# JokerJohn/DCReg

Hardware: AMD Instinct MI355X
Metric: ICP iterations/sec (higher is better)
Workload: dtype f64

## Files before the change

dcreg_amd/api.py:

```python
import ctypes as C
import math
import os

import numpy as np

_HERE = os.path.dirname(os.path.abspath(__file__))
LIB_PATH = os.environ.get("DCREG_LIB") or os.path.join(_HERE, "lib", "libdcreg_hip.so")

DETECTION = {"NONE_DETE": 0, "SCHUR_CONDITION_NUMBER": 1, "FULL_EVD_MIN_EIGENVALUE": 2,
             "EVD_SUB_CONDITION": 3, "FULL_SVD_CONDITION": 4}
HANDLING = {"NONE_HAND": 0, "STANDARD_REGULARIZATION": 1, "ADAPTIVE_REGULARIZATION": 2,
            "PRECONDITIONED_CG": 3, "SOLUTION_REMAPPING": 4, "TRUNCATED_SVD": 5}
METHODS = {
    "ME-SR": ("FULL_EVD_MIN_EIGENVALUE", "SOLUTION_REMAPPING"),
    "ME-TSVD": ("FULL_EVD_MIN_EIGENVALUE", "TRUNCATED_SVD"),
    "ME-TReg": ("FULL_EVD_MIN_EIGENVALUE", "STANDARD_REGULARIZATION"),
    "FCN-SR": ("FULL_SVD_CONDITION", "SOLUTION_REMAPPING"),
    "Ours": ("SCHUR_CONDITION_NUMBER", "PRECONDITIONED_CG"),
    "NONE": ("NONE_DETE", "NONE_HAND"),
}

OK, E_INVALID, E_NOMEM, E_DEVICE, E_STATE = 0, -1, -2, -3, -4
ROBUST = {"none": 0, "huber": 1, "cauchy": 2, "geman_mcclure": 3}
ROBUST_SCALE_RANGE = (1.0e-6, 1.0e6)
# ... 2240 lines not shown
    def hint_misalignment(self, metres):
        self._check(self._L.dcreg_hint_misalignment(self._h, float(metres)), "dcreg_hint_misalignment")

    def reset_warm_state(self, state_id):
        self._check(self._L.dcreg_reset_warm_state(self._h, int(state_id)), "dcreg_reset_warm_state")

    def launch_stats(self, reset=False):
        st = LaunchStats()
        self._check(self._L.dcreg_launch_stats_get(self._h, C.byref(st), int(reset)), "dcreg_launch_stats_get")
        return {k: int(getattr(st, k)) for k, _ in LaunchStats._fields_}

    def linearize_batch_warm(self, Rs, ts, state_ids, params=None, slot=0):
        params = params or default_lin_params()
        Rs = _f64(Rs).reshape(-1, 9)
        ts = _f64(ts).reshape(-1, 3)
        n = Rs.shape[0]
        ids = np.ascontiguousarray(state_ids, dtype=np.int32).reshape(n)
        outs = (LinOut * n)()
        self._check(self._L.dcreg_linearize_batch_begin_warm(self._h, slot, n, _dp(Rs), _dp(ts), ids.ctypes.data_as(C.POINTER(C.c_int32)),
                                                             C.byref(params)), "dcreg_linearize_batch_begin_warm")
        self._check(self._L.dcreg_linearize_batch_end(self._h, slot, outs), "dcreg_linearize_batch_end")
        return [self._out_dict(o) for o in outs]

    def linearize_begin(self, R, t, params=None, slot=0):
        params = params or default_lin_params()
        R = _f64(R).reshape(9); t = _f64(t).reshape(3)
        self._check(self._L.dcreg_linearize_batch_begin(self._h, slot, 1, _dp(R), _dp(t), C.byref(params)), "dcreg_linearize_batch_begin")

    def linearize_gated_begin(self, params=None, slot=0):
        params = params or default_lin_params()
        self._check(self._L.dcreg_linearize_gated_begin(self._h, slot, C.byref(params)), "dcreg_linearize_gated_begin")

    def gate_open(self, R, t):
        R = _f64(R).reshape(9); t = _f64(t).reshape(3)
        self._check(self._L.dcreg_linearize_gate_open(self._h, _dp(R), _dp(t)), "dcreg_linearize_gate_open")

    def gate_abort(self):
        self._check(self._L.dcreg_linearize_gate_abort(self._h), "dcreg_linearize_gate_abort")

    def linearize_end(self, slot=0):
        out = (LinOut * 1)()
        self._check(self._L.dcreg_linearize_batch_end(self._h, slot, out), "dcreg_linearize_batch_end")
        return self._out_dict(out[0])

    def knn(self, q, k=5, max_radius=0.0):
        q = _points(q, "knn")
        idx = np.empty((q.shape[0], k), np.int32)
        d2 = np.empty((q.shape[0], k), np.float32)
        self._check(self._L.dcreg_knn(self._h, q.ctypes.data_as(C.POINTER(C.c_float)), q.shape[0], q.shape[1], k, float(max_radius),
                                      idx.ctypes.data_as(C.POINTER(C.c_int32)), d2.ctypes.data_as(C.POINTER(C.c_float))), "dcreg_knn")
        return idx, d2

    def kdtree_build(self, leaf_size=16):
        self._check(self._L.dcreg_kdtree_build(self._h, int(leaf_size)), "dcreg_kdtree_build")
        d, l, ms = C.c_int32(), C.c_int32(), C.c_double()
        self._check(self._L.dcreg_kdtree_info(self._h, C.byref(d), C.byref(l), C.byref(ms)), "dcreg_kdtree_info")
        return d.value, l.value, ms.value

    def knn_timed(self, q, k=5, max_radius=0.0, index="grid", repeats=10):
        q = _points(q, "knn_timed")
        idx = np.empty((q.shape[0], k), np.int32)
        d2 = np.empty((q.shape[0], k), np.float32)
        ms = C.c_double()
        self._check(self._L.dcreg_knn_timed(self._h, q.ctypes.data_as(C.POINTER(C.c_float)), q.shape[0], q.shape[1], k, float(max_radius),
                                            {"grid": 0, "kdtree": 1, "grid_sweep": 2}[index], int(repeats), idx.ctypes.data_as(C.POINTER(C.c_int32)),
                                            d2.ctypes.data_as(C.POINTER(C.c_float)), C.byref(ms)), "dcreg_knn_timed")
        return idx, d2, ms.value

    def launch_series(self, reset=True, cap=1 << 20):
        lp = C.POINTER(C.c_int64)
        n = self._L.dcreg_launch_series(self._h, None, None, None, None, 0, 0)
        if n < 0:
            raise DcregError("dcreg_launch_series failed")
        n = min(n, cap)
        ms = np.empty(n, np.float64)
        se, rf, pt = np.empty(n, np.int64), np.empty(n, np.int64), np.empty(n, np.int64)
        adv = np.zeros(n, np.uint8)
        if hasattr(self._L, "dcreg_launch_series_passes"):
            self._L.dcreg_launch_series_passes(self._h, adv.ctypes.data_as(C.POINTER(C.c_uint8)), n)
        st = np.where((adv & 3) != 0, 1, 0).astype(np.uint8)
        if hasattr(self._L, "dcreg_launch_series_structure"):
            self._L.dcreg_launch_series_structure(self._h, st.ctypes.data_as(C.POINTER(C.c_uint8)), n)
        self._L.dcreg_launch_series(self._h, _dp(ms), se.ctypes.data_as(lp), rf.ctypes.data_as(lp), pt.ctypes.data_as(lp), n, int(reset))
        return {"ms": ms, "searched": se, "refitted": rf, "points": pt, "advanced": adv & 3, "one_wave": (adv >> 2) & 1, "structure": st}

    def team_pass_stamps(self):
        n = self._L.dcreg_team_pass_stamps(self._h, None, 0)
        if n <= 0:
            return np.zeros((0, 8), np.uint64)
        st = np.zeros((n + 1, 8), np.uint64)
        rc = self._L.dcreg_team_pass_stamps(self._h, st.ctypes.data_as(C.POINTER(C.c_uint64)), n + 1)
        if rc < 0:
            self._check(rc, "dcreg_team_pass_stamps")
        return st

    def roi_info(self):
        v = (C.c_double * 11)()
        self._L.dcreg_roi_info.argtypes = [C.c_void_p, C.POINTER(C.c_double)]
        self._check(self._L.dcreg_roi_info(self._h, v), "dcreg_roi_info")
        return {"box_min": [v[0], v[1], v[2]], "box_max": [v[3], v[4], v[5]], "points": int(v[6]), "cell": v[7], "windows_built": int(v[8]),
                "active": bool(v[9]), "whole_map_capped": bool(v[10])}

    def kernel_time(self, reset=False):
        ms, n = C.c_double(), C.c_int64()
        self._L.dcreg_kernel_time(self._h, C.byref(ms), C.byref(n), int(reset))
        return ms.value, n.value

    def icp_run(self, T0, method, cfg, log_capacity=None):
        return self._run_logged("dcreg_icp_run", T0, method, cfg, log_capacity)

    def icp_run_sharded(self, T0, method, cfg, n_source_total, reduce_rows, log_capacity=None):
        T0 = _f64(T0).reshape(4, 4)
        R0, t0 = np.ascontiguousarray(T0[:3, :3]).reshape(9), np.ascontiguousarray(T0[:3, 3])
        det, hand = METHODS[method] if isinstance(method, str) else method
        cap = cfg.max_iterations if log_capacity is None else log_capacity
        logs = (IterLog * max(cap, 1))()
        res = IcpResult()
        err = []

        def _cb(row_ptr, _user):
            try:
                reduce_rows(np.ctypeslib.as_array(row_ptr, shape=(32,)))
                return 0
            except Exception as e:
                err.append(e)
                return 1
        cb = REDUCE_FN(_cb)
        rc = self._L.dcreg_icp_run_sharded(self._h, _dp(R0), _dp(t0), DETECTION[det], HANDLING[hand], C.byref(cfg),
                                           int(n_source_total), cb, None, logs, cap, C.byref(res))
        if err:
            raise err[0]
        self._check(rc, "dcreg_icp_run_sharded")
        n = min(res.iterations, cap)
        if res.status == 1:
            n = min(res.iterations - 1, cap)
        return res, [logs[i] for i in range(max(n, 0))]

    def comm_init(self, id128, rank, world):
        buf = (C.c_char * 128).from_buffer_copy(bytes(id128))
        self._check(self._L.dcreg_comm_init(self._h, C.cast(buf, C.c_void_p), int(rank), int(world)), "dcreg_comm_init")

    def comm_allgather_sum(self, row):
        row = _f64(row, 32).copy()
        self._check(self._L.dcreg_comm_allgather_sum(self._h, _dp(row)), "dcreg_comm_allgather_sum")
        return row

    def icp_run_sharded_rccl(self, T0, method, cfg, n_source_total, log_capacity=None):
        return self._run_logged("dcreg_icp_run_sharded_rccl", T0, method, cfg, log_capacity, extra=(int(n_source_total),))

    def icp_run_euler(self, pose6d, method, cfg, log_capacity=None):
        p0 = _f64(pose6d, 6)
        det, hand = METHODS[method] if isinstance(method, str) else method
        cap = cfg.max_iterations if log_capacity is None else log_capacity
        logs = (IterLog * max(cap, 1))()
        res = IcpResult()
        pf = np.zeros(6)
        self._check(self._L.dcreg_icp_run_euler(self._h, _dp(p0), DETECTION[det], HANDLING[hand], C.byref(cfg), logs, cap,
                                                C.byref(res), _dp(pf)), "dcreg_icp_run_euler")
        return res, [logs[i] for i in range(max(min(res.iterations, cap), 0))], pf

    def icp_run_montecarlo(self, base_xyzrpy, seed, first_trial, trial_stride, n_trials, trans_amp, rot_amp_rad, method, cfg, slots=0):
        det, hand = METHODS[method]
        res = (TrialResult * max(int(n_trials), 1))()
        self._check(self._L.dcreg_icp_run_montecarlo(self._h, _dp(_f64(base_xyzrpy, 6)), int(seed), int(first_trial), int(trial_stride), int(n_trials),
                                                     float(trans_amp), float(rot_amp_rad), DETECTION[det], HANDLING[hand], C.byref(cfg), int(slots), res),
                    "dcreg_icp_run_montecarlo")
        return [res[i] for i in range(int(n_trials))]
# ... 346 lines not shown
```

dcreg_amd/csrc/device/context.hip:

```cpp
#include <algorithm>
#include <cmath>
#include <cstdarg>
#include <cstdio>
#include <cstdlib>
#include <chrono>
#include <cstring>
#include <string>
#include <vector>

#include <hip/hip_runtime.h>
#include <rocprim/device/device_radix_sort.hpp>
#include <rocprim/device/device_scan.hpp>

#include "../../../include/dcreg_debug.h"
#include "context.hpp"
#include "kernels.hpp"

namespace dcreg {

constexpr double kCountScale = 67108864.0;
constexpr size_t kSearchCountBytes = 64 * kCounterStride * sizeof(uint32_t);
static inline unsigned blocks_for(int64_t n, int bs) { return (unsigned)((n + bs - 1) / bs); }
static void drop_warm(dcreg_ctx *c);

// ... 1319 lines not shown
        const double Rx[9] = {1, 0, 0, 0, cr, -sr, 0, sr, cr}, dRx[9] = {0, 0, 0, 0, -sr, -cr, 0, cr, -sr};
        const double Ry[9] = {cp, 0, sp, 0, 1, 0, -sp, 0, cp}, dRy[9] = {-sp, 0, cp, 0, 0, 0, -cp, 0, -sp};
        const double Rz[9] = {cy, -sy, 0, sy, cy, 0, 0, 0, 1}, dRz[9] = {-sy, -cy, 0, cy, -sy, 0, 0, 0, 0};
        auto mul3 = [](const double *A, const double *B, const double *C3, double *out) {
            double T[9], O[9];
            for (int i = 0; i < 3; ++i) for (int j = 0; j < 3; ++j) { double s = 0; for (int k = 0; k < 3; ++k) s += A[i * 3 + k] * B[k * 3 + j]; T[i * 3 + j] = s; }
            for (int i = 0; i < 3; ++i) for (int j = 0; j < 3; ++j) { double s = 0; for (int k = 0; k < 3; ++k) s += T[i * 3 + k] * C3[k * 3 + j]; O[i * 3 + j] = s; }
            for (int i = 0; i < 3; ++i) { out[i * 3 + 0] = O[i * 3 + 1]; out[i * 3 + 1] = O[i * 3 + 2]; out[i * 3 + 2] = O[i * 3 + 0]; }
        };
        mul3(Rz, Ry, dRx, D); mul3(Rz, dRy, Rx, D + 9); mul3(dRz, Ry, Rx, D + 18);
    }
    HIP_TRY(c, hipMemcpyAsync(c->d_euler.data(), c->h_euler.data(), 27 * sizeof(double), hipMemcpyHostToDevice, c->stream));
    a.dR = c->d_euler.data();
    return DCREG_OK;
}

static void free_tmp(LinSlot &S) { S.tmp_dev.clear(); }

static void drop_warm(dcreg_ctx *c) {
    c->state_valid = false;
    c->nicp.warm_valid = false;
    c->nicp.drop_slots();
    c->adv_counts_dirty = true;
    std::fill(c->batch_state_valid.begin(), c->batch_state_valid.end(), (uint8_t)0);
}
static void gate_publish(dcreg_ctx *c, unsigned long long seq_word, const double *R, const double *t) {
    unsigned long long w[kGateWords];
    w[0] = seq_word;
    for (int k = 1; k < kGateWords - 1; ++k) w[k] = c->h_gate.data()->w[k];
    if (R) {
        std::memcpy(&w[1], R, 9 * sizeof(double));
        std::memcpy(&w[10], t, 3 * sizeof(double));
    }
    unsigned long long x = kGateSalt;
    for (int k = 0; k < kGateWords - 1; ++k) x ^= w[k];
    w[kGateWords - 1] = x;
    volatile unsigned long long *dst = c->h_gate.data()->w;
    for (int k = 1; k < kGateWords; ++k) dst[k] = w[k];
    __atomic_store_n(&c->h_gate.data()->w[0], w[0], __ATOMIC_RELEASE);
}
static void gate_call_off(dcreg_ctx *c) { gate_publish(c, (c->gate_seq << 1) | 1ull, nullptr, nullptr); }

static double pose_jump(const dcreg_ctx *c, const double *R9, const double *t3, const double *R, const double *t) {
    double dr = 0.0, dt = 0.0;
    for (int k = 0; k < 9; ++k) dr += (R9[k] - R[k]) * (R9[k] - R[k]);
    for (int k = 0; k < 3; ++k) dt += (t3[k] - t[k]) * (t3[k] - t[k]);
    return std::sqrt(dr) * c->src_radius + std::sqrt(dt);
}

static int estimate_dispatch_order(dcreg_ctx *c, const double *R9, const double *t3, int max_ring) {
    if (!c->d_group_est) HIP_TRY(c, c->d_group_est.alloc(kMaxGroups));
    PoseArg P{};
    for (int k = 0; k < 9; ++k) P.R[k] = R9[k];
    for (int k = 0; k < 3; ++k) P.t[k] = t3[k];
    const uint32_t ng = c->n_groups;
    const uint32_t lead = (blocks_for(c->n_src, kLinBlock) - ng * c->group_blocks) * (uint32_t)kLinBlock;
    hipLaunchKernelGGL(k_group_cost, dim3(ng), dim3(256), 0, c->stream, c->d_src.data() + lead, (uint32_t)c->n_src - lead, c->map.grid, P, c->group_blocks * (uint32_t)kLinBlock,
                       max_ring, c->d_group_est.data());
    float est[kMaxGroups];
    HIP_TRY(c, hipMemcpyAsync(est, c->d_group_est.data(), sizeof(float) * ng, hipMemcpyDeviceToHost, c->stream));
    HIP_TRY(c, hipStreamSynchronize(c->stream));
    uint32_t order[kMaxGroups];
    for (uint32_t k = 0; k < (uint32_t)kMaxGroups; ++k) order[k] = k;
    std::stable_sort(order, order + ng, [&](uint32_t x, uint32_t y) { return est[x] > est[y]; });
    for (uint32_t k = 0; k < (uint32_t)kMaxGroups; ++k) c->group_order[k] = (uint8_t)order[k];
    double sum = 0.0, mx = 0.0;
    for (uint32_t k = 0; k < ng; ++k) { sum += est[k]; mx = std::max(mx, (double)est[k]); }
    c->order_uneven = mx * ng > 1.3 * sum;
    std::memcpy(c->est_R, R9, sizeof(c->est_R)); std::memcpy(c->est_t, t3, sizeof(c->est_t));
    c->order_valid = true; c->est_launch = (int64_t)c->seq;
    return DCREG_OK;
}

struct LinLaunch {
    int slot, n_poses; const double *R9, *t3; const int32_t *state_ids, *frame_ids, *grid_ids; const dcreg_lin_params *p; dcreg_lin_debug *dbg;
    LinKind kind; int64_t n;
    dcreg_ctx::FrameSet *fs;
    dcreg_ctx::StateKey key; LinArgs a; DebugDev dd;
    PoseArg one;
    const PoseArg *d_poses;
    const uint2 *d_slices;
    const uint32_t *d_grid_ids;
    bool state_was_valid;
    bool own() const { return kind >= LinKind::single; }
    bool uses_state(const dcreg_ctx *c) const { return own() && c->opt_warm; }
};

static int lin_check(dcreg_ctx *c, LinLaunch &L) {
    const bool gated = L.kind == LinKind::gated;
    const dcreg_lin_debug *d = L.dbg;
    const bool stamps_only = d && d->stamps && !d->nn_idx && !d->nn_d2 && !d->flag && !d->normal && !d->r && !d->s && !d->stats;
    if (c->gate_slot >= 0) { c->fail("a gated linearisation still waits for its pose (dcreg_linearize_gate_open / _gate_abort first)"); return DCREG_E_STATE; }
    if (gated) {
        static const double eye[9] = {1, 0, 0, 0, 1, 0, 0, 0, 1}, zero[3] = {0, 0, 0};
        L.R9 = eye; L.t3 = zero; L.n_poses = 1; L.state_ids = nullptr; L.dbg = nullptr;
        if (!c->opt_spin) { c->fail("gated launches need the \"spin\" option (results through pinned flags)"); return DCREG_E_STATE; }
        if (c->opt_time_kernels > 0 && (c->launch_counter % (uint64_t)c->opt_time_kernels) == 0) {
            c->fail("the next launch is a timed one: not gated"); return DCREG_E_STATE;
        }
    }
    if (L.slot < 0 || L.slot >= dcreg_ctx::kLinSlots) { c->fail("invalid slot"); return DCREG_E_INVALID; }
    if (c->slots[L.slot].pending) { c->fail("slot %d still has a linearisation in flight", L.slot); return DCREG_E_STATE; }
    if (c->nicp.batch_pending()) { c->fail("a batched normal linearisation is still in flight (dcreg_normals_batch_end first)"); return DCREG_E_STATE; }
    if (!L.R9 || !L.t3 || L.n_poses < 1) { c->fail("null argument"); return DCREG_E_INVALID; }
    if (L.n_poses > 65535) { c->fail("at most 65535 poses per batched launch (grid.y limit), got %d", L.n_poses); return DCREG_E_INVALID; }
    if (!poses_finite(L.n_poses, L.R9, L.t3)) { c->fail("a pose with non-finite entries"); return DCREG_E_INVALID; }
    if (!L.grid_ids && c->map.n <= 0) { c->fail("KdTree/target index is not set up in context"); return DCREG_E_STATE; }
    L.fs = L.grid_ids ? &c->pair_src : &c->frames;
    if (L.grid_ids) {
        if (!L.frame_ids) { c->fail("pair launches name a source for every pose"); return DCREG_E_INVALID; }
        const dcreg_ctx::PairSet &ps = c->pairs;
        for (int i = 0; i < L.n_poses; ++i) {
            const int32_t t = L.grid_ids[i];
            if (t < 0 || t >= ps.n || !ps.built[(size_t)t]) { c->fail("pair target %d is not built", t); return DCREG_E_INVALID; }
        }
        if (!L.p || search_bound_sq(c, L.p->search_radius) != ps.radius_sq_f) { c->fail("the pair targets were built for another search radius"); return DCREG_E_INVALID; }
    }
    L.n = c->n_src;
    if (L.frame_ids) {
        if (!L.state_ids || L.dbg || gated) { c->fail("frame launches are batched product launches"); return DCREG_E_INVALID; }
        L.n = 0;
        for (int i = 0; i < L.n_poses; ++i) {
            const int32_t f = L.frame_ids[i];
            if (f < 0 || (size_t)f >= L.fs->slice.size() || L.fs->slice[(size_t)f].y == 0u) { c->fail("frame %d is not loaded or empty", f); return DCREG_E_INVALID; }
            L.n = std::max<int64_t>(L.n, L.fs->slice[(size_t)f].y);
        }
    } else
    if (c->n_src <= 0) { c->fail("measure cloud is not set"); return DCREG_E_STATE; }
    L.kind = L.grid_ids ? LinKind::pairs : L.frame_ids ? LinKind::frames : gated ? LinKind::gated : (L.n_poses > 1 || L.state_ids) ? LinKind::batch :
             !L.dbg ? LinKind::single : stamps_only ? LinKind::stamps : LinKind::dump;
    if (!L.p && !gated && (c->roi_active || roi_wanted(c))) { c->fail("null argument"); return DCREG_E_INVALID; }
    const dcreg_lin_params *p = L.p;
    if (!p || !(p->search_radius > 0.0)) { c->fail("invalid linearisation parameters"); return DCREG_E_INVALID; }
    if (p->k != 5 && p->k != 0) { c->fail("only k = 5 is supported (icp_test_runner.cpp:1722)"); return DCREG_E_INVALID; }
    if (p->parameterization != DCREG_PARAM_SO3 && p->parameterization != DCREG_PARAM_EULER && p->parameterization != DCREG_PARAM_EULER_EXACT) { c->fail("unknown parameterization"); return DCREG_E_INVALID; }
    if (L.state_ids && c->opt_warm) {
        const int64_t n_states = L.frame_ids ? L.fs->n_states : c->n_batch_states;
        std::vector<uint8_t> seen((size_t)std::max<int64_t>(n_states, 1), 0);
        for (int i = 0; i < L.n_poses; ++i) {
            const int32_t sid = L.state_ids[i];
            if (sid < 0) continue;
            if ((int64_t)sid >= n_states) { c->fail("warm state %d was not reserved (dcreg_reserve_warm_states: %lld)", sid, (long long)n_states); return DCREG_E_INVALID; }
            if (seen[(size_t)sid]) { c->fail("warm state %d is used by two poses of one launch", sid); return DCREG_E_INVALID; }
            seen[(size_t)sid] = 1;
        }
    }
    return DCREG_OK;
}

static bool order_wanted(const dcreg_ctx *c, const LinLaunch &L) {
    return c->opt_dispatch_order && L.own() && c->n_groups >= 2 && blocks_for(L.n, kLinBlock) > 4u * (uint32_t)c->n_cus &&
           c->hint_misalign > 0.5 * c->map.grid.h;
}

static LinPlan lin_plan(const dcreg_ctx *c, const LinLaunch &L, bool fresh) {
    LinPlan P;
    P.kind = L.kind; P.n_poses = L.n_poses; P.nbx = blocks_for(L.n, kLinBlock);
    P.n_chunks = (P.nbx + kChunk - 1) / kChunk;
    const bool fused = L.n_poses == 1 || P.n_chunks == 1;
    P.direct = fused && L.n_poses == 1 && P.nbx <= (uint32_t)kChunk && c->opt_one_wave < 2;
    P.n_rows = P.direct ? (size_t)P.nbx : (fused ? (size_t)P.n_chunks * (size_t)P.n_poses : (size_t)P.n_poses);
    const bool dbg = L.kind == LinKind::dump || L.kind == LinKind::stamps;
    P.use_cert = L.kind != LinKind::dump && c->opt_use_cert;
    P.ordered = order_wanted(c, L) && c->order_valid && c->order_uneven;
    const bool known = c->last_searched >= 0 && c->last_points == L.n;
    const double f = known ? (double)c->last_searched / (double)L.n : -1.0;
    if ((L.kind == LinKind::single || L.kind == LinKind::gated) && c->opt_warm && !fresh && P.use_cert && L.a.count_scale != 0.0) {
        constexpr double kAdvanceLo = 0.005, kAdvanceHi = 0.70;
        const bool adv = c->opt_advance >= 2 || (c->opt_advance == 1 && P.nbx >= (uint32_t)c->opt_advance_min_blocks && known && f >= kAdvanceLo && f <= kAdvanceHi);
        constexpr double kTeamPassMaxPoints = 16384.0, kTeamPassMinFrac = 0.5, kTeamPassMinCellPts = 3.0;
        const double per_cell = (double)c->map.n / (double)std::max<uint32_t>(c->map.occupied, 1u);
        const bool team = c->opt_team_pass >= 2 || (c->opt_team_pass == 1 && L.n <= (int64_t)kTeamPassMaxPoints && known && f >= kTeamPassMinFrac &&
                                                    per_cell >= kTeamPassMinCellPts);
        P.pass = team ? LinPass::team : adv ? LinPass::advance : LinPass::none;
    }
    bool one_wave = false;
    if (L.n_poses > 1)
        one_wave = fused && !dbg && (c->opt_one_wave >= 2 || (c->opt_one_wave_batches && (uint64_t)L.n_poses * P.nbx >= (uint64_t)c->opt_one_wave_min_blocks));
    else if (!P.direct && !dbg && P.pass != LinPass::team) {
        const bool most = !L.uses_state(c) || fresh || !P.use_cert || (known && (double)c->last_searched >= c->opt_one_wave_min_frac * (double)L.n);
        one_wave = c->opt_one_wave >= 2 || (c->opt_one_wave == 1 && P.nbx >= (uint32_t)c->opt_one_wave_min_blocks && P.pass != LinPass::advance && most &&
                                            c->hint_misalign > c->opt_one_wave_min_cells * c->map.grid.h);
    }
    P.gate_inside = L.kind == LinKind::gated && c->opt_gate_in_kernel && P.nbx <= (uint32_t)kChunk && P.pass != LinPass::advance;
    P.body = (P.gate_inside && P.pass != LinPass::team) ? LinBody::gated : L.kind == LinKind::stamps ? LinBody::stamps : L.kind == LinKind::dump ? LinBody::dump :
             one_wave ? LinBody::one_wave : fused ? LinBody::fused : LinBody::chunked;
    P.pass_rows = P.pass == LinPass::advance && c->opt_advance_fused != 0 && !P.direct && P.body == LinBody::fused;
    return P;
}

static int stage_poses(dcreg_ctx *c, LinSlot &S, LinLaunch &L) {
    const int64_t n_states = L.frame_ids ? L.fs->n_states : c->n_batch_states;
    std::vector<uint8_t> &state_valid = L.frame_ids ? L.fs->state_valid : c->batch_state_valid;
    dcreg_ctx::StateKey &states_key = L.frame_ids ? L.fs->key : c->batch_state_key;
    const bool use_states = L.state_ids && c->opt_warm && n_states > 0;
    if (use_states && !(L.key == states_key)) {
        std::fill(state_valid.begin(), state_valid.end(), (uint8_t)0);
        states_key = L.key;
    }
    const int n_poses = L.n_poses;
    const size_t bytes = (size_t)n_poses * sizeof(PoseArg) + (L.frame_ids ? (size_t)n_poses * sizeof(uint2) : 0) +
                         (L.grid_ids ? (size_t)n_poses * sizeof(uint32_t) : 0);
    if (bytes > S.d_poses.cap()) {
        S.h_poses.reset(); S.d_poses.reset();
        const size_t cap = std::max<size_t>(bytes, 256 * (sizeof(PoseArg) + sizeof(uint2) + sizeof(uint32_t)));
        HIP_TRY(c, S.h_poses.alloc(cap, hipHostMallocDefault));
        if (S.d_poses.alloc(cap) != hipSuccess) { c->fail("hipMalloc(%zu B) failed", cap); return DCREG_E_NOMEM; }
    }
    PoseArg *hp = (PoseArg *)S.h_poses.data();
    for (int i = 0; i < n_poses; ++i) {
        std::memcpy(hp[i].R, L.R9 + 9 * i, sizeof(hp[i].R)); std::memcpy(hp[i].t, L.t3 + 3 * i, sizeof(hp[i].t));
        const bool has = use_states && L.state_ids[i] >= 0;
        hp[i].state = has ? (uint32_t)L.state_ids[i] : kNoIdx;
        hp[i].fresh = (has && state_valid[(size_t)L.state_ids[i]] != 0) ? 0u : 1u;
        if (has) state_valid[(size_t)L.state_ids[i]] = 1;
    }
    if (L.frame_ids) {
        uint2 *hs = (uint2 *)(S.h_poses.data() + (size_t)n_poses * sizeof(PoseArg));
        for (int i = 0; i < n_poses; ++i) hs[i] = L.fs->slice[(size_t)L.frame_ids[i]];
        L.d_slices = (const uint2 *)(S.d_poses.data() + (size_t)n_poses * sizeof(PoseArg));
    }
    if (L.grid_ids) {
        const size_t at = (size_t)n_poses * (sizeof(PoseArg) + sizeof(uint2));
        std::memcpy(S.h_poses.data() + at, L.grid_ids, sizeof(uint32_t) * (size_t)n_poses);
        L.d_grid_ids = (const uint32_t *)(S.d_poses.data() + at);
    }
    HIP_TRY(c, hipMemcpyAsync(S.d_poses.data(), S.h_poses.data(), bytes, hipMemcpyHostToDevice, c->stream));
    L.d_poses = (const PoseArg *)S.d_poses.data();
    if (use_states && L.frame_ids) { L.a.state = L.fs->state.data(); L.a.state_stride = (uint32_t)L.fs->state_stride; }
    else if (use_states) { L.a.state = c->d_state_batch.data(); L.a.state_stride = (uint32_t)c->state_batch_stride; }
    return DCREG_OK;
}

static int lin_reserve(dcreg_ctx *c, LinSlot &S, LinLaunch &L, const LinPlan &P) {
    if (int rc = stage_euler(c, L.p, L.a)) return rc;
    if (S.d_partials.ensure(c, (size_t)P.n_poses * P.nbx * kSlots * (P.one_wave() ? kLinBlock / kWave : 1))) return DCREG_E_NOMEM;
    if (P.fused()) {
        const size_t had = S.d_tickets.cap();
        if (S.d_tickets.ensure(c, (size_t)P.n_chunks * (size_t)P.n_poses * kCounterStride)) return DCREG_E_NOMEM;
        if (S.d_tickets.cap() != had || S.tickets_dirty) {
            HIP_TRY(c, hipMemsetAsync(S.d_tickets.data(), 0, sizeof(unsigned int) * S.d_tickets.cap(), c->stream));
            S.tickets_dirty = false;
        }
    }
    if (P.n_rows * kSlots > S.h_out.cap()) {
        const size_t cap = std::max<size_t>(P.n_rows, 64) * kSlots;
        HIP_TRY(c, S.h_out.alloc(cap, hipHostMallocMapped | hipHostMallocCoherent));
        std::memset(S.h_out.data(), 0, cap * sizeof(double));
        std::fill(S.row_chk.begin(), S.row_chk.end(), 0ull);
    }
    if (L.kind == LinKind::gated) {
        if (!c->h_gate) {
            PinnedBuf<GateHost> hg; DevBuf<PoseArg> dp; DevBuf<uint32_t> da; DevBuf<GateDev> gd;
            bool ok = hg.alloc(1, hipHostMallocMapped | hipHostMallocCoherent) == hipSuccess;
            ok = ok && dp.alloc(1) == hipSuccess && da.alloc(1) == hipSuccess;
            ok = ok && gd.alloc(1) == hipSuccess && hipMemsetAsync(gd.data(), 0, sizeof(GateDev), c->stream) == hipSuccess;
            if (!ok) {
                c->state_valid = L.state_was_valid;
                c->fail("allocating the launch gate failed");
                return DCREG_E_NOMEM;
            }
            std::memset(hg.data(), 0, sizeof(GateHost));
            c->h_gate = std::move(hg); c->d_gate_pose = std::move(dp); c->d_gate_abort = std::move(da); c->d_gate_dev = std::move(gd);
        }
        L.d_poses = c->d_gate_pose.data();
    }
    if (int rc = L.own() ? DCREG_OK : stage_poses(c, S, L)) return rc;
    if (P.pass != LinPass::none && !P.pass_rows) {
        const size_t had = c->d_adv_counts.cap();
        if (c->d_adv_counts.ensure(c, (size_t)kCounterStride * P.nbx)) return DCREG_E_NOMEM;
        if (c->d_adv_counts.cap() != had || c->adv_counts_dirty) {
            HIP_TRY(c, hipMemsetAsync(c->d_adv_counts.data(), 0, sizeof(uint32_t) * c->d_adv_counts.cap(), c->stream));
            c->adv_counts_dirty = false;
        }
        L.a.adv_counts = c->d_adv_counts.data();
    }
    if (P.pass == LinPass::team && c->opt_team_stamps) {
        const uint32_t n_tiles = blocks_for(L.n, kTeamTile);
        if (c->d_team_stamps.ensure(c, (size_t)8 * (n_tiles + 1))) return DCREG_E_NOMEM;
        HIP_TRY(c, hipMemsetAsync(c->d_team_stamps.data(), 0, sizeof(unsigned long long) * 8 * (n_tiles + 1), c->stream));
        c->team_stamps_n = n_tiles;
    }
    free_tmp(S);
    if (L.dbg) {
        const dcreg_lin_debug *dbg = L.dbg; const size_t n = (size_t)L.n; DebugDev &dd = L.dd;
        bool oom = false;
        auto alloc = [&](size_t bytes, int fill) -> void * {
            DevBuf<unsigned char> b;
            if (b.alloc(bytes) != hipSuccess) { oom = true; return nullptr; }
            (void)hipMemsetAsync(b.data(), fill, bytes, c->stream);
            S.tmp_dev.push_back(std::move(b));
            return S.tmp_dev.back().data();
        };
        if (dbg->nn_idx) dd.nn_idx = (int32_t *)alloc(sizeof(int32_t) * 5 * n, 0xFF);
        if (dbg->nn_d2) dd.nn_d2 = (float *)alloc(sizeof(float) * 5 * n, 0);
        if (dbg->flag) dd.flag = (uint8_t *)alloc(n, 0);
        if (dbg->normal) dd.normal = (double *)alloc(sizeof(double) * 3 * n, 0);
        if (dbg->r) dd.r = (double *)alloc(sizeof(double) * n, 0);
        if (dbg->s) dd.s = (double *)alloc(sizeof(double) * n, 0);
        if (dbg->stats) dd.stats = (uint32_t *)alloc(sizeof(uint32_t) * n, 0);
        if (dbg->stamps) dd.stamps = (unsigned long long *)alloc(sizeof(unsigned long long) * 8 * (kLinBlock / 64) * (size_t)P.nbx, 0);
        if (oom) { free_tmp(S); drop_warm(c); c->fail("hipMalloc of the debug dump buffers failed"); return DCREG_E_NOMEM; }
    }
    L.a.use_cert = P.use_cert ? 1 : 0;
    L.a.search_count = c->opt_count_searches ? c->d_search_count.data() : nullptr;
    L.a.group_blocks = std::max<uint32_t>(c->group_blocks, 1u); L.a.n_groups = P.ordered ? c->n_groups : 0u;
    std::memcpy(L.a.group_order, c->group_order, sizeof(L.a.group_order));
    return DCREG_OK;
}

using LinKernel = decltype(&k_lin<0, true, true>);
template <bool FAST, bool SLICE = false, bool GRIDS = false>
static LinKernel lin_kernel(const LinPlan &P) {
    if constexpr (!SLICE) {
        if (P.kind == LinKind::pairs) return lin_kernel<FAST, true, true>(P);
        if (P.kind == LinKind::frames) return lin_kernel<FAST, true>(P);
        if (P.body == LinBody::gated) return k_lin<0, true, FAST, true>;
        if (P.body == LinBody::stamps) return k_lin<2, true, FAST>;
        if (P.body == LinBody::dump) return k_lin<1, true, FAST>;
    }
    if (P.one_wave()) return k_lin<0, true, FAST, false, true, SLICE, GRIDS>;
    return P.fused() ? k_lin<0, true, FAST, false, false, SLICE, GRIDS> : k_lin<0, false, FAST, false, false, SLICE, GRIDS>;
}

template <bool FAST>
static int lin_queue(dcreg_ctx *c, LinSlot &S, LinLaunch &L, const LinPlan &P) {
    const bool gated = L.kind == LinKind::gated, team = P.pass == LinPass::team, slice = L.kind == LinKind::frames || L.kind == LinKind::pairs;
    const uint32_t n = (uint32_t)L.n;
    const unsigned long long seq = ++c->seq;
    FinArgs fin{S.d_tickets.data(), S.h_out.dev(), seq, P.direct ? 1u : 0u, P.n_chunks};
    if (P.fused()) S.tickets_dirty = true;
    bool timed = c->opt_time_kernels > 0 && (c->launch_counter++ % (uint64_t)c->opt_time_kernels) == 0;
    if (timed && !S.ev0) timed = false;
    const uint32_t *abort_flag = nullptr;
    auto bail = [&](const char *what, hipError_t e) {
        if (e == hipSuccess) return DCREG_OK;
        free_tmp(S);
        if (gated) gate_call_off(c);
        drop_warm(c);
        c->fail("%s failed: %s", what, hipGetErrorString(e));
        return DCREG_E_DEVICE;
    };
    auto record = [&](hipEvent_t ev) { return bail("hipEventRecord", timed ? hipEventRecord(ev, c->stream) : hipSuccess); };
    GateArgs gt{nullptr, nullptr, 0ull, nullptr, nullptr, 0u};
    const PoseArg *lin_poses = L.d_poses;
    if (gated) {
        const unsigned long long want = ++c->gate_seq;
        if (P.gate_inside) {
            gt = GateArgs{c->h_gate.dev(), c->d_gate_dev.data(), want, team ? c->d_gate_pose.data() : nullptr, team ? c->d_gate_abort.data() : nullptr, L.one.fresh};
            if (team) abort_flag = c->d_gate_abort.data();
            else lin_poses = nullptr;
        } else {
            hipLaunchKernelGGL(k_gate, dim3(1), dim3(64), 0, c->stream, c->h_gate.dev(), want, c->d_gate_pose.data(), L.one.fresh, c->d_gate_abort.data());
            abort_flag = c->d_gate_abort.data();
        }
    }
    if (int rc = record(S.ev0)) return rc;
    if (P.pass == LinPass::advance) {
        const auto pass = P.pass_rows ? k_advance<FAST, true> : k_advance<FAST, false>;
        hipLaunchKernelGGL(pass, dim3(blocks_for(L.n, kAdvTile)), dim3(kLinBlock), 0, c->stream, c->d_src.data(), n, c->map.grid, L.one, L.d_poses, L.a,
                           P.pass_rows ? nullptr : c->d_adv_counts.data(), abort_flag, S.d_partials.data(), P.nbx, fin);
    }
    if (team) {
        const auto pass = P.gate_inside ? k_advance_team<FAST, true> : k_advance_team<FAST>;
        hipLaunchKernelGGL(pass, dim3(blocks_for(L.n, kTeamTile)), dim3(kWave), 0, c->stream, c->d_src.data(), n, c->map.grid, L.one, P.gate_inside ? nullptr : L.d_poses,
                           L.a, c->d_adv_counts.data(), P.gate_inside ? nullptr : abort_flag, c->opt_team_stamps ? c->d_team_stamps.data() : nullptr, gt);
    }
    if (P.pass != LinPass::none) {
        if (int rc = bail(team ? "team advance pass launch" : "advance pass launch", hipGetLastError())) return rc;
        c->n_advance_launches += 1;
    }
    const bool one = P.one_wave(); const auto lin = lin_kernel<FAST>(P);
    if (!P.pass_rows)
    hipLaunchKernelGGL(lin, dim3(one ? P.nbx * (kLinBlock / kWave) : P.nbx, (unsigned)P.n_poses), dim3(one ? kWave : kLinBlock), 0, c->stream,
                       slice ? L.fs->src.data() : c->d_src.data(), n, c->map.grid, L.one, lin_poses, L.a, S.d_partials.data(), P.nbx, fin, L.dd, abort_flag, gt,
                       L.d_slices, L.kind == LinKind::pairs ? c->pairs.d_grids.data() : nullptr, L.d_grid_ids);
    if (one)
        hipLaunchKernelGGL(slice ? k_sum_tiles<true> : k_sum_tiles<false>, dim3(P.n_chunks, (unsigned)P.n_poses), dim3(kLinBlock), 0, c->stream, S.d_partials.data(),
                           P.nbx, S.h_out.dev(), seq, abort_flag, L.d_slices);
    if (int rc = bail("linearisation kernel launch", hipGetLastError())) return rc;
    if (!P.fused()) {
        hipLaunchKernelGGL(slice ? k_finalize<true> : k_finalize<false>, dim3((unsigned)P.n_poses), dim3(kLinBlock), 0, c->stream, S.d_partials.data(), P.nbx,
                           S.h_out.dev(), seq, L.d_slices);
        if (int rc = bail("k_finalize launch", hipGetLastError())) return rc;
    }
    if (int rc = record(S.ev1)) return rc;
    if (const dcreg_lin_debug *dbg = L.dbg) {
        const DebugDev &dd = L.dd;
        hipError_t ce = hipSuccess;
        auto back = [&](void *dst, const void *srcp, size_t bytes) { if (ce == hipSuccess && srcp) ce = hipMemcpyAsync(dst, srcp, bytes, hipMemcpyDeviceToHost, c->stream); };
        back(dbg->nn_idx, dd.nn_idx, sizeof(int32_t) * 5 * n);
        back(dbg->nn_d2, dd.nn_d2, sizeof(float) * 5 * n);
        back(dbg->flag, dd.flag, (size_t)n);
        back(dbg->normal, dd.normal, sizeof(double) * 3 * n);
        back(dbg->r, dd.r, sizeof(double) * n);
        back(dbg->s, dd.s, sizeof(double) * n);
        back(dbg->stats, dd.stats, sizeof(uint32_t) * n);
        back(dbg->stamps, dd.stamps, sizeof(unsigned long long) * 8 * (kLinBlock / 64) * (size_t)P.nbx);
        if (ce != hipSuccess) { (void)hipStreamSynchronize(c->stream); return bail("copying the debug dump back", ce); }
    }
    c->n_launches += 1; c->n_poses_launched += P.n_poses; c->n_points_launched += (int64_t)P.n_poses * L.n;
    if (L.uses_state(c)) c->state_valid = true;
    S.pending = true; S.plan = P; S.timed = timed; S.seq = seq; S.sync = L.dbg != nullptr;
    S.coded = L.a.count_scale != 0.0;
    if (gated) {
        c->gate_slot = L.slot;
        c->gate_uses_state = L.uses_state(c); c->gate_state_was_valid = L.state_was_valid;
    }
    return DCREG_OK;
}

static int linearize_begin(dcreg_ctx *c, int slot, int n_poses, const double *R9, const double *t3, const int32_t *state_ids,
                           const dcreg_lin_params *p, dcreg_lin_debug *dbg_host, bool gated = false, const int32_t *frame_ids = nullptr,
                           const int32_t *grid_ids = nullptr) {
    if (!c) return DCREG_E_INVALID;
    LinLaunch L{slot, n_poses, R9, t3, state_ids, frame_ids, grid_ids, p, dbg_host, gated ? LinKind::gated : LinKind::single};
    if (int rc = lin_check(c, L)) return rc;
    if (c->need_set_device) { HIP_TRY(c, hipSetDevice(c->device)); }
    if (gated && c->roi_active && roi_pad_for(c, p->search_radius) > c->roi_pad) (void)roi_deactivate(c);
    if (!gated && L.kind != LinKind::pairs && (c->roi_active || roi_wanted(c))) {
        const bool product = L.kind == LinKind::single || L.kind == LinKind::stamps;
        if (int rc = product ? roi_ensure(c, L.R9, L.t3, p->search_radius) : roi_deactivate(c)) return rc;
    }
    L.a = make_lin_args(c, p, L.kind != LinKind::pairs, L.n);
    const LinArgs &a = L.a;
    L.key.radius_sq = a.radius_sq; L.key.max_thick_sq = a.max_thick_sq; L.key.min_norm = a.min_norm;
    L.key.radius_sq_f = a.radius_sq_f; L.key.cert_r_out = a.cert_r_out; L.key.cert_r_in = a.cert_r_in; L.key.fast_plane = c->opt_fast_plane ? 1 : 0;
    if (L.own() && !gated) {
        const double jump = c->last_pose_valid ? pose_jump(c, L.R9, L.t3, c->last_R, c->last_t) : 1e300;
        if (c->hint_unknown && jump <= 0.5 * c->map.grid.h) c->hint_misalign = c->hint_last;
        if (jump > 0.5 * c->map.grid.h) { c->last_searched = c->n_src; c->last_points = c->last_searched; }
        c->hint_unknown = false;
        std::memcpy(c->last_R, L.R9, sizeof(c->last_R)); std::memcpy(c->last_t, L.t3, sizeof(c->last_t));
        c->last_pose_valid = true;
    }
    if (!gated && order_wanted(c, L)) {
        bool stale = !c->order_valid;
        if (!stale && (int64_t)c->seq - c->est_launch >= 16)
            stale = pose_jump(c, L.R9, L.t3, c->est_R, c->est_t) > c->map.grid.h;
        if (int rc = stale ? estimate_dispatch_order(c, L.R9, L.t3, a.max_ring) : DCREG_OK) return rc;
    }
    if (L.uses_state(c) && !(L.key == c->state_key)) { c->state_valid = false; c->state_key = L.key; }
    L.state_was_valid = c->state_valid;
    L.one.state = kNoIdx; L.one.fresh = 1;
    if (L.own()) {
        std::memcpy(L.one.R, L.R9, sizeof(L.one.R)); std::memcpy(L.one.t, L.t3, sizeof(L.one.t));
        if (c->opt_warm) {
            const size_t stride = ((size_t)L.n + 63) & ~(size_t)63;
            if (!c->state_valid || c->state_stride != stride) {
                if (c->d_state.ensure(c, kStateRows * stride)) return DCREG_E_NOMEM;
                c->state_stride = stride; c->state_valid = false;
            }
            L.one.state = 0; L.one.fresh = c->state_valid ? 0u : 1u;
            L.a.state = c->d_state.data(); L.a.state_stride = (uint32_t)c->state_stride;
        }
    }
    const LinPlan P = lin_plan(c, L, L.one.fresh != 0u);
    LinSlot &S = c->slots[slot];
    if (int rc = lin_reserve(c, S, L, P)) return rc;
    return c->opt_fast_plane ? lin_queue<true>(c, S, L, P) : lin_queue<false>(c, S, L, P);
}

static int wait_rows(dcreg_ctx *c, LinSlot &S) {
    using Clk = std::chrono::steady_clock;
    Clk::time_point t0;
    bool clocked = false;
    const uint64_t every = c->opt_wait_seconds < 1.0 ? ((1ull << 6) - 1) : ((1ull << 20) - 1);
    static const struct Mults { unsigned long long m[kSlots]; Mults() { for (int k = 0; k < kSlots; ++k) m[k] = row_check_mult(k); } } mults;
    auto arrived = [&](size_t i) {
        unsigned long long v[kSlots];
        asm volatile("" ::: "memory");
        std::memcpy(v, (const void *)(S.h_out.data() + i * kSlots), sizeof(v));
        unsigned long long c0 = S.seq * mults.m[31], c1 = 0, c2 = 0, c3 = 0;
        for (int k = 0; k < 28; k += 4) { c0 += v[k] * mults.m[k]; c1 += v[k + 1] * mults.m[k + 1]; c2 += v[k + 2] * mults.m[k + 2]; c3 += v[k + 3] * mults.m[k + 3]; }
        c0 += v[28] * mults.m[28]; c1 += v[29] * mults.m[29]; c2 += v[30] * mults.m[30];
        if (c0 + c1 + c2 + c3 != v[31]) return false;
        std::memcpy(S.h_rows.data() + i * kSlots, v, sizeof(v));
        S.row_chk[i] = v[31];
        return true;
    };
    auto touched = [&](size_t i) {
        return __atomic_load_n((const unsigned long long *)(S.h_out.data() + i * kSlots) + 31, __ATOMIC_RELAXED) != S.row_chk[i];
    };
    S.h_rows.resize(S.plan.n_rows * kSlots);
    S.row_done.assign(S.plan.n_rows, 0);
    if (S.row_chk.size() < S.plan.n_rows) S.row_chk.resize(S.plan.n_rows, 0ull);
    size_t pending = S.plan.n_rows;
    uint64_t spins = 0;
    while (pending) {
        for (size_t i = 0; i < S.plan.n_rows; ++i)
            if (!S.row_done[i] && touched(i) && arrived(i)) { S.row_done[i] = 1; --pending; }
        if (!pending) break;
        __builtin_ia32_pause();
        if ((++spins & every) != 0) continue;
        if (!clocked) { t0 = Clk::now(); clocked = true; continue; }
        if (std::chrono::duration<double>(Clk::now() - t0).count() < c->opt_wait_seconds) continue;
        if (c->gate_slot >= 0) (void)dcreg_linearize_gate_abort(c);
        const hipError_t e = hipStreamSynchronize(c->stream);
        if (e != hipSuccess) { c->fail("device fault while waiting for a linearisation: %s", hipGetErrorString(e)); return DCREG_E_DEVICE; }
        for (size_t i = 0; i < S.plan.n_rows; ++i)
            if (!S.row_done[i]) {
                if (!arrived(i)) { c->fail("linearisation result never arrived"); return DCREG_E_DEVICE; }
                S.row_done[i] = 1; --pending;
            }
    }
    return DCREG_OK;
}

static int linearize_end(dcreg_ctx *c, int slot, dcreg_lin_out *outs) {
    if (!c) return DCREG_E_INVALID;
    if (slot < 0 || slot >= dcreg_ctx::kLinSlots) { c->fail("invalid slot"); return DCREG_E_INVALID; }
    LinSlot &S = c->slots[slot];
    if (!S.pending) { c->fail("slot %d has no linearisation in flight", slot); return DCREG_E_STATE; }
    if (!outs) { c->fail("null argument"); return DCREG_E_INVALID; }
    S.pending = false;
    int rc = DCREG_OK;
    if (S.sync || !c->opt_spin) {
        const hipError_t e = hipStreamSynchronize(c->stream);
        if (e != hipSuccess) { c->fail("hipStreamSynchronize failed: %s", hipGetErrorString(e)); rc = DCREG_E_DEVICE; }
        if (rc == DCREG_OK && S.sync) { const hipError_t e2 = hipGetLastError(); if (e2 != hipSuccess) { c->fail("%s", hipGetErrorString(e2)); rc = DCREG_E_DEVICE; } }
        if (rc == DCREG_OK) rc = wait_rows(c, S);
    } else {
        rc = wait_rows(c, S);
    }
    free_tmp(S);
    if (rc != DCREG_OK) { drop_warm(c); return rc; }
// ... 144 lines not shown
        return DCREG_E_DEVICE;
    }
    c->stream = c->own_stream;
    for (LinSlot &S : c->slots)
        if (hipEventCreate(&S.ev0) != hipSuccess || hipEventCreate(&S.ev1) != hipSuccess) { S.ev0 = S.ev1 = nullptr; }
    *out = c;
    return DCREG_OK;
}

void dcreg_backend_destroy(dcreg_ctx *c) {
    if (!c) return;
    (void)dcreg_comm_destroy(c);
    (void)hipSetDevice(c->device);
    (void)dcreg_linearize_gate_abort(c);
    (void)hipStreamSynchronize(c->stream);
    if (c->h_stage_ev) (void)hipEventDestroy(c->h_stage_ev);
    if (c->null_ev) (void)hipEventDestroy(c->null_ev);
    kdtree_free(c->kd); c->kd = nullptr;
    for (LinSlot &S : c->slots) {
        if (S.ev0) (void)hipEventDestroy(S.ev0);
        if (S.ev1) (void)hipEventDestroy(S.ev1);
    }
    for (auto &B : c->nicp.batch) if (B.done) (void)hipEventDestroy(B.done);
    (void)hipEventDestroy(c->ev0); (void)hipEventDestroy(c->ev1);
    (void)hipStreamDestroy(c->own_stream);
    delete c;
}

const char *dcreg_last_error(const dcreg_ctx *c) { return c ? c->err : "null context"; }
void dcreg_set_error_message(dcreg_ctx *c, const char *msg) { if (c && msg) c->fail("%s", msg); }

int dcreg_set_stream(dcreg_ctx *c, void *s) {
    if (!c) return DCREG_E_INVALID;
    if (int rc = refuse_in_flight(c)) return rc;
    (void)hipStreamSynchronize(c->stream);
    c->stream = s ? (hipStream_t)s : c->own_stream;
    return DCREG_OK;
}

int dcreg_set_option(dcreg_ctx *c, const char *key, double v) {
    if (!c || !key) return DCREG_E_INVALID;
    const std::string k(key);
    if (k == "cell") c->opt_cell = v;
    else if (k == "cell_factor") c->opt_cell_factor = v > 0.1 ? v : 2.0;
    else if (k == "use_certificates") c->opt_use_cert = v != 0.0;
    else if (k == "count_searches") {
        if (v != 0.0 && !c->d_search_count) {
            HIP_TRY(c, c->d_search_count.alloc(kSearchCountBytes / sizeof(unsigned long long)));
            HIP_TRY(c, hipMemsetAsync(c->d_search_count.data(), 0, kSearchCountBytes, c->stream));
        }
        c->opt_count_searches = v != 0.0;
    }
    else if (k == "cert_margin" || k == "cert_inflate" || k == "warm_start" || k == "fast_plane_fit") {
        if (c->gate_slot >= 0) { c->fail("a gated linearisation is queued: open or abort it before changing \"%s\"", key); return DCREG_E_STATE; }
        if (k == "cert_margin") c->opt_cert_margin = v >= 1e-4 ? std::min(v, 1.0) : 1e-4;
        else if (k == "cert_inflate") c->opt_cert_inflate = v >= 0.0 ? std::min(v, 1.0) : 0.0;
        else if (k == "warm_start") c->opt_warm = v != 0.0;
        else c->opt_fast_plane = v != 0.0;
        drop_warm(c);
    }
    else if (k == "wait_seconds") c->opt_wait_seconds = v > 0.0 ? v : 30.0;
    else if (k == "x_subdiv") { int sx = 1; while (sx < 16 && (double)(sx * 2) <= v) sx *= 2; c->opt_x_subdiv = sx; }
    else if (k == "time_kernels") { c->opt_time_kernels = v > 0.0 ? (int)v : 0; c->launch_counter = 0; }
    else if (k == "record_launches") { c->opt_record_launches = v != 0.0; if (v == 0.0) c->launch_series.clear(); }
    else if (k == "curve_x_scale") c->opt_curve_x_scale = (v > 0.0 && v <= 1.0) ? v : 1.0;
    else if (k == "roi_index") { c->opt_roi_index = (int)std::min(std::max(v, 0.0), 2.0); c->roi_built = false; }
    else if (k == "roi_margin") { c->opt_roi_margin = std::min(std::max(v, 0.0), 1.0e6); c->roi_built = false; }
    else if (k == "pair_max_table_entries") c->opt_pair_max_table_entries = (int64_t)std::min(std::max(v, 4096.0), 2147483648.0);
    else if (k == "pairs_max_bytes") c->opt_pairs_max_bytes = std::max(v, 0.0);
    else if (k == "visibility_max_bytes") c->opt_visibility_max_bytes = std::max(v, 0.0);
    else if (k == "visibility_order") c->opt_visibility_order = (int)v;
    else if (k == "max_table_entries") c->opt_max_table_entries = (int64_t)std::min(std::max(v, 1048576.0), 2147483648.0);
    else if (k == "advance") c->opt_advance = (int)v;
    else if (k == "advance_fused") c->opt_advance_fused = (int)v;
    else if (k == "one_wave") c->opt_one_wave = (int)v;
    else if (k == "one_wave_batches") c->opt_one_wave_batches = v != 0.0;
    else if (k == "one_wave_min_frac") c->opt_one_wave_min_frac = v;
    else if (k == "one_wave_min_cells") c->opt_one_wave_min_cells = v;
    else if (k == "one_wave_min_blocks") c->opt_one_wave_min_blocks = (int)v;
    else if (k == "gate_in_kernel") c->opt_gate_in_kernel = v != 0.0;
    else if (k == "team_stamps") c->opt_team_stamps = v != 0.0;
    else if (k == "team_pass") c->opt_team_pass = (int)v;
    else if (k == "advance_min_blocks") c->opt_advance_min_blocks = (int)v;
    else if (k == "team_search") c->opt_team_max = (int)v;
    else if (k == "spin") c->opt_spin = v != 0.0;
    else if (k == "far_bound") c->opt_far_bound = v != 0.0;
    else if (k == "dispatch_order") { c->opt_dispatch_order = v != 0.0; c->order_valid = false; }
    else if (k == "keep_source_order") c->opt_keep_source_order = v != 0.0;
    else if (k == "gap_field") c->opt_gap_field = v != 0.0;
    else if (k == "map_update") c->opt_map_update = v != 0.0 ? 1 : 0;
    else if (k == "normals_follow") c->opt_normals_follow = v != 0.0 ? 1 : 0;
    else if (k == "normals_follow_full_share") c->opt_normals_follow_full_share = std::min(std::max(v, 0.0), 1.0);
    else if (k == "gicp_epsilon") {
        if (!(v >= 1.0e-6 && v <= 1.0)) { c->fail("gicp_epsilon is %g: 1e-6 .. 1 expected", v); return DCREG_E_INVALID; }
        c->opt_gicp_epsilon = v;
    }
    else if (k == "robust_kernel") {
        if (!(v == (double)DCREG_ROBUST_NONE || v == (double)DCREG_ROBUST_HUBER || v == (double)DCREG_ROBUST_CAUCHY || v == (double)DCREG_ROBUST_GEMAN_MCCLURE)) {
            c->fail("robust_kernel is %g: 0 (none), 1 (Huber), 2 (Cauchy) or 3 (Geman-McClure) expected", v); return DCREG_E_INVALID;
        }
        c->opt_robust_kernel = (int)v;
    }
    else if (k == "robust_scale" || k == "gicp_robust_scale") {
        if (!(v >= 1.0e-6 && v <= 1.0e6)) { c->fail("%s is %g: 1e-6 .. 1e6 expected", key, v); return DCREG_E_INVALID; }
        (k == "robust_scale" ? c->opt_robust_scale : c->opt_gicp_robust_scale) = v;
    }
    else if (k == "voxels_source_cov") {
        if (!(v == 0.0 || v == 1.0)) { c->fail("voxels_source_cov is %g: 0 or 1 expected", v); return DCREG_E_INVALID; }
        c->opt_voxels_source_cov = (int)v;
    }
    else if (k == "voxels_neighbors") {
        if (!(v == 1.0 || v == 7.0 || v == 27.0)) { c->fail("voxels_neighbors is %g: 1, 7 or 27 expected", v); return DCREG_E_INVALID; }
        c->opt_voxels_neighbors = (int)v;
    }
    else if (k == "map_grow_margin") c->opt_map_grow_margin = std::min(std::max(v, 0.0), 1.0e4);
    else { c->fail("unknown option '%s'", key); return DCREG_E_INVALID; }
    return DCREG_OK;
}

int dcreg_set_target(dcreg_ctx *c, const float *xyz, int64_t n, int64_t stride, double r) { return set_target(c, xyz, n, stride, r, false); }
int dcreg_set_target_device(dcreg_ctx *c, const float *xyz, int64_t n, int64_t stride, double r) { return set_target(c, xyz, n, stride, r, true); }
int dcreg_target_insert(dcreg_ctx *c, const float *xyz, int64_t n, int64_t stride, const double R[9], const double t[3], double min_spacing,
                        dcreg_map_update *info) {
    return map_insert(c, xyz, n, stride, false, false, R, t, min_spacing, info);
}
int dcreg_target_insert_device(dcreg_ctx *c, const float *d_xyz, int64_t n, int64_t stride, const double R[9], const double t[3], double min_spacing,
                               dcreg_map_update *info) {
    return map_insert(c, d_xyz, n, stride, true, false, R, t, min_spacing, info);
}
int dcreg_target_insert_source(dcreg_ctx *c, const double R[9], const double t[3], double min_spacing, dcreg_map_update *info) {
    return map_insert(c, nullptr, 0, 3, false, true, R, t, min_spacing, info);
}
int dcreg_target_crop(dcreg_ctx *c, const double lo[3], const double hi[3], dcreg_map_update *info) { return map_crop(c, lo, hi, info); }
int dcreg_target_get(const dcreg_ctx *c, float *xyz_out, int64_t capacity_points) { return target_get(c, xyz_out, capacity_points); }
int dcreg_debug_index_check(dcreg_ctx *c, int64_t mismatches[5]) {
    if (!c || !mismatches) return DCREG_E_INVALID;
    if (int rc = refuse_in_flight(c)) return rc;
    if (whole_map(c).n <= 0) { c->fail("no target"); return DCREG_E_STATE; }
    HIP_TRY(c, hipSetDevice(c->device));
    return index_check(c, mismatches);
}
int dcreg_set_source(dcreg_ctx *c, const float *xyz, int64_t n, int64_t stride) { return set_source(c, xyz, n, stride, false); }
int dcreg_set_source_device(dcreg_ctx *c, const float *xyz, int64_t n, int64_t stride) { return set_source(c, xyz, n, stride, true); }

static void voxel_info(dcreg_voxel_info *info, const VoxelResult &r) {
    if (info) { info->n_in = r.n_in; info->n_finite = r.n_finite; info->n_voxels = r.n_voxels; info->n_out = r.n_out; }
}
static int set_cloud_voxel(dcreg_ctx *c, const float *xyz, int64_t n, int64_t stride, bool on_device, const dcreg_voxel_params *p, bool target,
                           double radius_hint, dcreg_voxel_info *info, DeskewRun *dsk = nullptr, dcreg_deskew_info *dinfo = nullptr,
                           const GatherRun *gat = nullptr) {
    if (!c) return DCREG_E_INVALID;
    if (int rc = refuse_in_flight(c)) return rc;
    if (n <= 0) { c->fail("%s cloud is null or empty", target ? "target" : "measure"); return DCREG_E_INVALID; }
    HIP_TRY(c, hipSetDevice(c->device));
    const int64_t off[2] = {0, n};
    VoxelResult r;
    int rc = voxel_pass(c, 1, xyz, off, stride, on_device, p, true, r, dsk, gat);
    if (rc) return rc;
    voxel_info(info, r);
    if (dsk) deskew_info(*dsk, n, dinfo);
    if (r.n_out <= 0) { c->fail("no point of the %s cloud is left after the voxel pass", target ? "target" : "measure"); return DCREG_E_INVALID; }
    if (target) {
        const double box[6] = {r.mn[0], r.mn[1], r.mn[2], r.mx[0], r.mx[1], r.mx[2]};
        return target_commit(c, r.n_out, box, radius_hint);
    }
    return source_commit(c, r.n_out, r.mn, r.mx, true);
// ... 176 lines not shown
    if (n_states < 0) { c->fail("negative state count"); return DCREG_E_INVALID; }
    for (const LinSlot &S : c->slots) if (S.pending) { c->fail("a linearisation is still in flight"); return DCREG_E_STATE; }
    fs.n_states = 0;
    fs.state_valid.clear();
    if (n_states == 0 || fs.max_points <= 0) return DCREG_OK;
    HIP_TRY(c, hipSetDevice(c->device));
    const size_t stride = ((size_t)fs.max_points + 63) & ~(size_t)63;
    if (fs.state.ensure(c, kStateRows * stride * (size_t)n_states)) return DCREG_E_NOMEM;
    fs.state_stride = stride;
    fs.n_states = n_states;
    fs.state_valid.assign((size_t)n_states, 0);
    return DCREG_OK;
}
static int frames_reset_state(dcreg_ctx *c, dcreg_ctx::FrameSet &fs, int64_t state_id) {
    if (state_id < 0 || state_id >= fs.n_states) { c->fail("frame state %lld was not reserved", (long long)state_id); return DCREG_E_INVALID; }
    fs.state_valid[(size_t)state_id] = 0;
    return DCREG_OK;
}
int dcreg_frames_reserve_states(dcreg_ctx *c, int64_t n_states) { return c ? frames_reserve_states(c, c->frames, n_states) : DCREG_E_INVALID; }
int dcreg_frames_reset_state(dcreg_ctx *c, int64_t state_id) { return c ? frames_reset_state(c, c->frames, state_id) : DCREG_E_INVALID; }
static int pairs_plan(dcreg_ctx *c, int n_pairs, const int64_t *tgt_offsets, int64_t stride_floats, double extra, int32_t *batch_end, int *n_batches,
                      bool voxels = false) {
    if (!c || n_pairs < 0 || !tgt_offsets || !batch_end || !n_batches) return DCREG_E_INVALID;
    const double budget = pairs_budget(c);
    int nb = 0;
    double bytes = 0.0;
    int64_t pts = 0;
    for (int p = 0; p < n_pairs; ++p) {
        const int64_t m = tgt_offsets[p + 1] - tgt_offsets[p];
        const double b = voxels ? pair_voxel_target_bytes(m, stride_floats) : pair_target_bytes(c, m, stride_floats, extra);
        if (p > 0 && (bytes + b > budget || pts + m >= ((int64_t)1 << 31) - 1)) { batch_end[nb++] = p; bytes = 0.0; pts = 0; }
        bytes += b; pts += m;
    }
    if (n_pairs > 0) batch_end[nb++] = n_pairs;
    *n_batches = nb;
    return DCREG_OK;
}
int dcreg_pairs_plan(dcreg_ctx *c, int n_pairs, const int64_t *tgt_offsets, int64_t stride_floats, int32_t *batch_end, int *n_batches) {
    return pairs_plan(c, n_pairs, tgt_offsets, stride_floats, 0.0, batch_end, n_batches);
}
int dcreg_pairs_plan_normals(dcreg_ctx *c, int n_pairs, const int64_t *tgt_offsets, int64_t stride_floats, int32_t *batch_end, int *n_batches) {
    return pairs_plan(c, n_pairs, tgt_offsets, stride_floats, 32.0, batch_end, n_batches);
}
int dcreg_pairs_plan_voxels(dcreg_ctx *c, int n_pairs, const int64_t *tgt_offsets, int64_t stride_floats, int32_t *batch_end, int *n_batches) {
    return pairs_plan(c, n_pairs, tgt_offsets, stride_floats, 0.0, batch_end, n_batches, true);
}
int dcreg_pairs_sources_load(dcreg_ctx *c, int n_pairs, const float *xyz, const int64_t *src_offsets, int64_t stride_floats) {
    if (!c) return DCREG_E_INVALID;
    if (int rc = refuse_in_flight(c)) return rc;
    if (c->nicp.slots_for == dcreg_ctx::NormalIcpBufs::SlotsFor::pairs) c->nicp.drop_slots();
    c->pair_src.normals_kept = false;
    return frames_load(c, c->pair_src, n_pairs, xyz, src_offsets, stride_floats);
}
int dcreg_pairs_build(dcreg_ctx *c, int n_targets, const float *xyz, const int64_t *tgt_offsets, int64_t stride_floats, double search_radius) {
    if (!c) return DCREG_E_INVALID;
    if (int rc = refuse_in_flight(c)) return rc;
    return pairs_build(c, n_targets, xyz, tgt_offsets, stride_floats, search_radius);
}
int dcreg_pairs_reserve_states(dcreg_ctx *c, int64_t n_states) { return c ? frames_reserve_states(c, c->pair_src, n_states) : DCREG_E_INVALID; }
int dcreg_pairs_reset_state(dcreg_ctx *c, int64_t state_id) { return c ? frames_reset_state(c, c->pair_src, state_id) : DCREG_E_INVALID; }
int dcreg_pairs_batch_begin(dcreg_ctx *c, int slot, int n, const double *R9, const double *t3, const int32_t *state_ids, const int32_t *source_ids,
                            const int32_t *target_ids, const dcreg_lin_params *p) {
    if (c && (!source_ids || !state_ids || !target_ids)) { c->fail("null argument"); return DCREG_E_INVALID; }
    return linearize_begin(c, slot, n, R9, t3, state_ids, p, nullptr, false, source_ids, target_ids);
}
int dcreg_frames_batch_begin(dcreg_ctx *c, int slot, int n, const double *R9, const double *t3, const int32_t *state_ids, const int32_t *frame_ids,
                             const dcreg_lin_params *p) {
    if (c && (!frame_ids || !state_ids)) { c->fail("null argument"); return DCREG_E_INVALID; }
    return linearize_begin(c, slot, n, R9, t3, state_ids, p, nullptr, false, frame_ids);
}
int dcreg_linearize_gated_begin(dcreg_ctx *c, int slot, const dcreg_lin_params *p) {
    return linearize_begin(c, slot, 1, nullptr, nullptr, nullptr, p, nullptr, true);
}
int dcreg_linearize_gate_open(dcreg_ctx *c, const double R[9], const double t[3]) {
    if (!c) return DCREG_E_INVALID;
    if (c->gate_slot < 0 || !R || !t) { c->fail("no gated linearisation waits for a pose"); return DCREG_E_STATE; }
    if (!poses_finite(1, R, t)) { c->fail("a pose with non-finite entries: the gate still waits"); return DCREG_E_INVALID; }
    if (c->roi_active && !roi_covers(c, R, t, c->roi_pad)) {
        (void)dcreg_linearize_gate_abort(c);
        c->fail("the pose left the window of the map the queued launch was built on: launch called off");
        return DCREG_E_STATE;
    }
    gate_publish(c, c->gate_seq << 1, R, t);
    std::memcpy(c->last_R, R, sizeof(c->last_R)); std::memcpy(c->last_t, t, sizeof(c->last_t));
    c->last_pose_valid = true;
    c->gate_slot = -1;
    return DCREG_OK;
}
int dcreg_linearize_gate_abort(dcreg_ctx *c) {
    if (!c) return DCREG_E_INVALID;
    if (c->gate_slot < 0) return DCREG_OK;
    gate_call_off(c);
    LinSlot &S = c->slots[c->gate_slot];
    S.pending = false;
    free_tmp(S);
    if (c->gate_uses_state) c->state_valid = c->gate_state_was_valid;
    c->gate_slot = -1;
    return DCREG_OK;
}
int dcreg_linearize_debug(dcreg_ctx *c, const double R[9], const double t[3], const dcreg_lin_params *p, dcreg_lin_out *out, dcreg_lin_debug *dbg) {
    return launch_linearize(c, 1, R, t, p, out, dbg);
}

int dcreg_knn(dcreg_ctx *c, const float *q, int64_t n, int64_t stride, int k, double max_radius, int32_t *idx, float *d2) {
    if (!c) return DCREG_E_INVALID;
    if (int rc = refuse_in_flight(c)) return rc;
    if (!q || !idx || !d2 || n < 0 || (k != 1 && k != 5)) { c->fail("invalid k-NN arguments (k must be 1 or 5)"); return DCREG_E_INVALID; }
    (void)roi_deactivate(c);
    if (c->map.n <= 0) { c->fail("target index is not set"); return DCREG_E_STATE; }
    if (n == 0) return DCREG_OK;
    HIP_TRY(c, hipSetDevice(c->device));
    int rc = upload_cloud(c, q, n, stride, false, c->d_aligned);
    if (rc) return rc;
    if (c->d_nn_idx.ensure(c, (size_t)n * k) || c->d_nn_d2.ensure(c, (size_t)n * k)) return DCREG_E_NOMEM;
    rc = launch_knn(c, c->map.grid, c->d_aligned.data(), n, k, max_radius, nullptr, c->d_nn_idx.data(), c->d_nn_d2.data());
    if (rc) return rc;
    HIP_TRY(c, hipMemcpyAsync(idx, c->d_nn_idx.data(), sizeof(int32_t) * (size_t)n * k, hipMemcpyDeviceToHost, c->stream));
    HIP_TRY(c, hipMemcpyAsync(d2, c->d_nn_d2.data(), sizeof(float) * (size_t)n * k, hipMemcpyDeviceToHost, c->stream));
    HIP_TRY(c, hipStreamSynchronize(c->stream));
    return DCREG_OK;
}

int dcreg_index_info_get(const dcreg_ctx *c, dcreg_index_info *info) {
    if (!c || !info) return DCREG_E_INVALID;
    const IndexSet &w = whole_map(c);
    const dcreg::GridDev &g = w.grid;
    info->cell = g.h;
    info->origin[0] = g.ox; info->origin[1] = g.oy; info->origin[2] = g.oz;
    info->dims[0] = g.nx; info->dims[1] = g.ny; info->dims[2] = g.nz;
    info->n_cells = w.n_cells; info->n_target = w.n;
    info->n_source = c->n_src; info->max_ring = c->last_max_ring;
    return DCREG_OK;
}

int dcreg_roi_info(const dcreg_ctx *c, double info[11]) {
    if (!c || !info) return DCREG_E_INVALID;
    for (int a = 0; a < 3; ++a) { info[a] = c->roi_lo[a]; info[3 + a] = c->roi_hi[a]; }
    const bool have = c->roi_built && !c->roi_empty;
    const IndexSet &win = c->roi_active ? c->map : c->roi_store;
    info[6] = have ? (double)win.n : 0.0;
    info[7] = have ? win.grid.h : 0.0;
    info[8] = (double)c->roi_rebuilds; info[9] = c->roi_active ? 1.0 : 0.0; info[10] = c->whole_capped ? 1.0 : 0.0;
    return DCREG_OK;
}

int dcreg_launch_stats_get(dcreg_ctx *c, dcreg_launch_stats *st, int reset) {
    if (!c || !st) return DCREG_E_INVALID;
    if (c->opt_count_searches && c->d_search_count) if (int rc = refuse_in_flight(c)) return rc;
    st->launches = c->n_launches; st->poses = c->n_poses_launched; st->points = c->n_points_launched;
    st->points_searched = -1; st->points_team = -1;
    if (c->opt_count_searches && c->d_search_count) {
        std::vector<unsigned long long> v(kSearchCountBytes / sizeof(unsigned long long));
        HIP_TRY(c, hipMemcpyAsync(v.data(), c->d_search_count.data(), kSearchCountBytes, hipMemcpyDeviceToHost, c->stream));
        HIP_TRY(c, hipStreamSynchronize(c->stream));
        unsigned long long tot = 0, team = 0;
        for (size_t k = 0; k < v.size(); k += kCounterStride / 2) { tot += v[k]; team += v[k + 1]; }
        st->points_searched = (int64_t)tot;
        st->points_team = (int64_t)team;
        if (reset) HIP_TRY(c, hipMemsetAsync(c->d_search_count.data(), 0, kSearchCountBytes, c->stream));
    }
    if (reset) { c->n_launches = 0; c->n_poses_launched = 0; c->n_points_launched = 0; }
    return DCREG_OK;
}

int dcreg_launch_series(dcreg_ctx *c, double *ms, int64_t *searched, int64_t *refitted, int64_t *points, int64_t cap, int reset) {
    if (!c || cap < 0) return -1;
    const int64_t n = std::min<int64_t>(cap, (int64_t)c->launch_series.size());
    for (int64_t i = 0; i < n; ++i) {
        const dcreg_ctx::LaunchRec &r = c->launch_series[(size_t)i];
        if (ms) ms[i] = r.ms;
        if (searched) searched[i] = r.searched;
        if (refitted) refitted[i] = r.refitted;
        if (points) points[i] = r.points;
    }
    const int64_t total = (int64_t)c->launch_series.size();
    if (reset) c->launch_series.clear();
    return (int)std::min<int64_t>(total, 0x7FFFFFFF);
}

// ... 50 lines not shown
```

dcreg_amd/csrc/device/context.hpp:

```cpp
#pragma once
#include <hip/hip_runtime.h>

#include <algorithm>
#include <chrono>
#include <cmath>
#include <cstdint>
#include <cstring>
#include <functional>
#include <utility>
#include <vector>

#include "../../../include/dcreg.h"
#include "kernels.hpp"

struct dcreg_lin_params;
struct dcreg_lin_out;
struct dcreg_lin_debug;

#define HIP_TRY(ctx, expr)                                                                       \
    do {                                                                                         \
        hipError_t e__ = (expr);                                                                 \
        if (e__ != hipSuccess) {                                                                 \
            (ctx)->fail("%s failed: %s (%s:%d)", #expr, hipGetErrorString(e__), __FILE__, __LINE__); \
            return DCREG_E_DEVICE;                                                               \
// ... 37 lines not shown
    PinnedBuf &operator=(const PinnedBuf &) = delete;
    PinnedBuf(PinnedBuf &&o) noexcept { swap(o); }
    PinnedBuf &operator=(PinnedBuf &&o) noexcept { if (this != &o) { reset(); swap(o); } return *this; }
    ~PinnedBuf() { reset(); }
    T *data() const { return p_; }
    T *dev() const { return d_; }
    size_t cap() const { return cap_; }
    explicit operator bool() const { return p_ != nullptr; }
    void swap(PinnedBuf &o) noexcept { std::swap(p_, o.p_); std::swap(d_, o.d_); std::swap(cap_, o.cap_); }
    void reset() { if (p_) (void)hipHostFree(p_); p_ = d_ = nullptr; cap_ = 0; }
    hipError_t alloc(size_t n, unsigned flags) {
        reset();
        hipError_t e = hipHostMalloc((void **)&p_, n * sizeof(T), flags);
        if (e != hipSuccess) { p_ = nullptr; return e; }
        if (flags & hipHostMallocMapped) e = hipHostGetDevicePointer((void **)&d_, p_, 0);
        if (e == hipSuccess) cap_ = n;
        return e;
    }
private:
    T *p_ = nullptr, *d_ = nullptr;
    size_t cap_ = 0;
};

namespace dcreg {
struct DeskewCloud {
    double xi[6];
    double t_begin, t_end, ref;
    int from_data;
    int pad_;
};
struct PathCloud {
    int64_t first_seg;
    int n_seg;
    int pad_;
    double s_first, s_last;
    double E[12];
};
struct PathSeg {
    double xi[6];
    double G[12];
    double s0, len;
};
struct KfMember {
    uint32_t start, src;
    double pose[12];
};
struct VisMember {
    uint32_t start, src, img, pad_;
    double pose[12];
};
__device__ __forceinline__ uint32_t seg_of(const int64_t *__restrict__ off, int n_clouds, int64_t i) {
    int lo = 0, hi = n_clouds;
    while (lo < hi) {
        const int mid = (lo + hi + 1) >> 1;
        if (off[mid] <= i) lo = mid; else hi = mid - 1;
    }
    return (uint32_t)lo;
}
}

namespace dcreg {
struct OneNnGrid {
    GridDev g;
    int max_ring;
    uint32_t normals_first;
};
struct PairVoxMap {
    uint32_t first, base, mask, n_kept;
    long long mn[3], mx[3];
};
}

enum class LinKind : uint8_t { batch, frames, pairs, single, gated, dump, stamps };
enum class LinPass : uint8_t { none, advance, team };
enum class LinBody : uint8_t { chunked, fused, one_wave, gated, dump, stamps };
struct LinPlan {
    LinKind kind = LinKind::single; LinPass pass = LinPass::none; LinBody body = LinBody::fused;
    int n_poses = 0; uint32_t nbx = 0, n_chunks = 0;
    size_t n_rows = 0;
    bool direct = false;
    bool gate_inside = false;
    bool pass_rows = false;
    bool ordered = false, use_cert = true;
    bool fused() const { return body != LinBody::chunked; }
    bool one_wave() const { return body == LinBody::one_wave; }
    int passes() const { return (int)pass | (one_wave() ? 4 : 0); }
    int structure() const { return pass_rows ? 2 : pass != LinPass::none ? 1 : 0; }
};

struct LinSlot {
    DevBuf<double> d_partials;
    PinnedBuf<unsigned char> h_poses;
    DevBuf<unsigned char> d_poses;
    PinnedBuf<double> h_out;
    std::vector<double> h_rows;
    DevBuf<unsigned int> d_tickets;
    bool tickets_dirty = false;
    std::vector<DevBuf<unsigned char>> tmp_dev;
    bool pending = false, timed = false, sync = false;
    LinPlan plan;
    std::vector<uint8_t> row_done;
    std::vector<unsigned long long> row_chk;
    unsigned long long seq = 0;
    hipEvent_t ev0 = nullptr, ev1 = nullptr;
    bool coded = false;
};

struct dcreg_ctx {
    int device = 0;
    hipStream_t own_stream = nullptr, stream = nullptr;
    hipEvent_t ev0 = nullptr, ev1 = nullptr;
    char err[512] = {0};

    struct IndexSet {
        DevBuf<float4> raw; int64_t n = 0;
        DevBuf<float4> sorted;
        DevBuf<uint32_t> cell_start;
        dcreg::GridDev grid{}; int64_t n_cells = 0; uint32_t occupied = 0;
        DevBuf<uint8_t> gap;
        DevBuf<uint32_t> owner, ymask;
    };
    IndexSet map;
    double radius_hint = 0.0;
    int last_max_ring = 0;
    IndexSet map_alt;
    DevBuf<float4> d_map_q, d_map_new;
    DevBuf<uint32_t> d_upd;
    DevBuf<uint8_t> d_fgap;
    DevBuf<uint32_t> d_fown;
    double tgt_box[6] = {};
    double build_per_cell = 0.0;
    int opt_map_update = 1;
    int opt_normals_follow = 0;
    double opt_normals_follow_full_share = 0.25;
    double opt_map_grow_margin = 20.0;

    IndexSet roi_store;
    bool roi_active = false;
    bool roi_built = false;
    bool roi_empty = false;
    int opt_roi_index = 1;
    double opt_roi_margin = 20.0;
    bool whole_capped = false;
    bool last_build_capped = false;
    double roi_lo[3] = {}, roi_hi[3] = {}, roi_pad = 0.0;
    double src_mn[3] = {}, src_mx[3] = {};
    int64_t roi_rebuilds = 0;

    IndexSet aux;
    bool aux_valid = false;

    int64_t n_src = 0;
    DevBuf<float4> d_src_raw;
    DevBuf<float4> d_src;
    DevBuf<uint32_t> d_state;
    size_t state_stride = 0;
    bool state_valid = false;
    struct StateKey {
        double radius_sq = -1.0, max_thick_sq = 0.0, min_norm = 0.0;
        float radius_sq_f = 0.f, cert_r_out = 0.f, cert_r_in = 0.f;
        int fast_plane = -1;
        bool operator==(const StateKey &o) const {
            return radius_sq == o.radius_sq && max_thick_sq == o.max_thick_sq && min_norm == o.min_norm && radius_sq_f == o.radius_sq_f &&
                   cert_r_out == o.cert_r_out && cert_r_in == o.cert_r_in && fast_plane == o.fast_plane;
        }
    };
    StateKey state_key, batch_state_key;
    double src_radius = 0.0;
    DevBuf<uint32_t> d_state_batch;
    size_t state_batch_stride = 0;
// ... 116 lines not shown
        DevBuf<float> reach; bool from_keep = false;
        dcreg_normal_params keep_params{};
        DevBuf<float4> normals_alt, f_list;
        DevBuf<float> reach_alt;
        DevBuf<uint32_t> f_bits, f_flag;
        dcreg_normals_follow_info follow{};
        DevBuf<uint32_t> warm; bool warm_valid = false;
        DevBuf<double> partials, d_out;
        DevBuf<unsigned char> dbg;
        struct BatchSlot {
            DevBuf<double> partials, d_out;
            PinnedBuf<unsigned char> h_poses;
            DevBuf<unsigned char> d_poses;
            PinnedBuf<double> h_out;
            hipEvent_t done = nullptr;
            int n_poses = 0;
            bool pending = false;
            std::vector<int32_t> ids;
        };
        BatchSlot batch[2];
        DevBuf<uint32_t> slots;
        size_t slot_stride = 0;
        int64_t n_slots = 0;
        enum class SlotsFor : uint8_t { source, frames, pairs };
        SlotsFor slots_for = SlotsFor::source;
        std::vector<uint8_t> slot_valid;
        bool batch_pending() const { return batch[0].pending || batch[1].pending; }
        void drop_slots() { std::fill(slot_valid.begin(), slot_valid.end(), (uint8_t)0); }
    };
    NormalIcpBufs nicp;
    struct GicpBufs {
        DevBuf<float4> src_normals; bool src_kept = false;
        DevBuf<float4> tmp;
    };
    GicpBufs gicp;
    struct VoxelMapBufs {
        DevBuf<float4> recs, tmp;
        DevBuf<uint64_t> vkeys, t_keys;
        DevBuf<uint32_t> t_vals;
        DevBuf<unsigned long long> cls;
        bool kept = false;
        int64_t n_kept = 0;
        uint32_t mask = 0;
        long long mn[3] = {}, mx[3] = {};
        double leaf = 0.0;
    };
    VoxelMapBufs vmap;
    int opt_voxels_source_cov = 0;
    int opt_voxels_neighbors = 1;
    double opt_gicp_epsilon = 1.0e-3;
    int opt_robust_kernel = 0;
    double opt_robust_scale = 0.1;
    double opt_gicp_robust_scale = 1.0;
    double opt_visibility_max_bytes = 268435456.0;
    int opt_visibility_order = 1;
    int64_t opt_pair_max_table_entries = (int64_t)1 << 24;
    double opt_pairs_max_bytes = 0.0;
    PinnedBuf<double> h_euler;
    DevBuf<double> d_euler;
    DevBuf<unsigned long long> d_search_count;

    DevBuf<float> d_stage;
    PinnedBuf<float> h_stage; hipEvent_t h_stage_ev = nullptr; bool h_stage_busy = false;
    hipEvent_t null_ev = nullptr;
    DevBuf<uint32_t> d_keys, d_keys2, d_vals, d_vals2;
    DevBuf<uint64_t> d_mkeys, d_mkeys2;
    DevBuf<uint32_t> d_scratch;
    DevBuf<char> sort_tmp;

    PinnedBuf<dcreg::GateHost> h_gate;
    DevBuf<dcreg::PoseArg> d_gate_pose;
    DevBuf<uint32_t> d_gate_abort;
    DevBuf<dcreg::GateDev> d_gate_dev;
    bool opt_gate_in_kernel = true;
    int opt_one_wave = 1;
    bool opt_one_wave_batches = true;
    double opt_one_wave_min_frac = 0.5;
    double opt_one_wave_min_cells = 1.5;
    int opt_one_wave_min_blocks = 1024;
    unsigned long long gate_seq = 0;
    int gate_slot = -1;
    bool gate_uses_state = false;
    bool gate_state_was_valid = false;
    static constexpr int kLinSlots = 2;
    LinSlot slots[kLinSlots];

    DevBuf<float4> d_aligned;
    DevBuf<int32_t> d_nn_idx;
    DevBuf<float> d_nn_d2;
    DevBuf<double> d_p2p_part;

    void *comm = nullptr;
    int comm_rank = 0, comm_world = 0;
    DevBuf<double> d_xrow, d_xall;
    PinnedBuf<double> h_xrow, h_xall;

    double opt_cell = 0.0, opt_cell_factor = 2.0;
    int opt_x_subdiv = 8;
    bool opt_use_cert = true;
    bool opt_count_searches = false;
    double opt_cert_inflate = 0.005;
    double opt_cert_margin = 0.05;
    int opt_time_kernels = 0;
    uint64_t launch_counter = 0;
    double opt_wait_seconds = 30.0;
    bool opt_spin = true;
    bool need_set_device = true;
    unsigned long long seq = 0;
    bool opt_fast_plane = true;
    bool opt_gap_field = true;
    bool opt_far_bound = true;
    bool opt_keep_source_order = false;
    bool opt_dispatch_order = true;
    uint8_t group_order[256] = {}; DevBuf<float> d_group_est;
    uint32_t group_blocks = 0, n_groups = 0;
    int n_cus = 256;
    void *kd = nullptr;
    bool order_valid = false;
    bool order_uneven = false;
    double est_R[9] = {}, est_t[3] = {};
    int64_t est_launch = 0;
    double hint_misalign = 1e300;
    bool hint_unknown = false;
    double hint_last = 1e300, last_R[9] = {}, last_t[3] = {};
    bool last_pose_valid = false;
    double opt_curve_x_scale = 1.0;
    int64_t opt_max_table_entries = (int64_t)1 << 30;
    int opt_advance = 1;
    int opt_advance_fused = 1;
    int opt_advance_min_blocks = 2048;
    int opt_team_pass = 1;
    bool opt_team_stamps = false;
    DevBuf<unsigned long long> d_team_stamps; uint32_t team_stamps_n = 0;
    DevBuf<uint32_t> d_adv_counts; bool adv_counts_dirty = true;
    int64_t n_advance_launches = 0;
    int opt_team_max = 7;
    bool opt_warm = true;
    int64_t n_launches = 0, n_poses_launched = 0, n_points_launched = 0;
    double kernel_ms_total = 0.0;
    int64_t kernel_launches = 0;
    int64_t last_searched = -1, last_refitted = -1, last_points = 0;
    struct LaunchRec { double ms; int64_t searched, refitted, points; int advanced, structure; };
    bool opt_record_launches = false;
    std::vector<LaunchRec> launch_series;

    struct PairVoxBufs {
        DevBuf<float4> recs, tmp;
        DevBuf<uint64_t> vkeys, t_keys;
        DevBuf<uint32_t> t_vals, d_words;
        DevBuf<unsigned long long> d_cnt;
        DevBuf<dcreg::PairVoxMap> d_maps;
        std::vector<dcreg::PairVoxMap> maps;
        int n = 0;
        double leaf = 0.0;
    };
    PairVoxBufs pvox;

    void fail(const char *fmt, ...);
};

template <typename T>
int DevBuf<T>::ensure(dcreg_ctx *c, size_t need, const char *why) {
    if (holds(need)) return DCREG_OK;
    const size_t n = std::max<size_t>(need, 1);
    const hipError_t e = alloc(n);
    if (e != hipSuccess) {
        (void)hipGetLastError();
        if (why) c->fail("hipMalloc(%zu B) failed %s", n * sizeof(T), why);
        else c->fail("hipMalloc(%zu B) failed: %s", n * sizeof(T), hipGetErrorString(e));
        return DCREG_E_NOMEM;
    }
    return DCREG_OK;
}

template <typename T>
int DevBuf<T>::grow_keep(dcreg_ctx *c, size_t need, size_t keep) {
    if (holds(need)) return DCREG_OK;
    DevBuf fresh;
    const size_t n = std::max(need, cap_ + cap_ / 2);
    if (fresh.alloc(n) != hipSuccess) {
        (void)hipGetLastError();
        c->fail("hipMalloc(%zu B) failed while growing the map", n * sizeof(T));
        return DCREG_E_NOMEM;
    }
    if (p_ && keep) HIP_TRY(c, hipMemcpyAsync(fresh.p_, p_, keep * sizeof(T), hipMemcpyDeviceToDevice, c->stream));
    HIP_TRY(c, hipStreamSynchronize(c->stream));
    swap(fresh);
    return DCREG_OK;
}

namespace dcreg {

int launch_linearize(dcreg_ctx *c, int n_poses, const double *R9, const double *t3, const dcreg_lin_params *p,
                     dcreg_lin_out *outs, dcreg_lin_debug *dbg_host);
void kdtree_free(void *kd);
int roi_ensure(dcreg_ctx *c, const double *R, const double *t, double search_radius);
inline bool finite_n(const double *v, int64_t n) {
    for (int64_t k = 0; k < n; ++k) if (!std::isfinite(v[k])) return false;
    return true;
}
struct DumpField { void *host; size_t bytes; void *dev; };
int rows_run(dcreg_ctx *c, dcreg_lin_out *out, const DumpField *fields, int n_fields, const std::function<void(double *partials, uint32_t nb)> &launch);
struct OneNnBound { double radius_sq; float bound_f; int max_ring; };
int one_nn_check(dcreg_ctx *c, const double *R, const double *t, const dcreg_lin_params *p, const dcreg_lin_out *out, const char *what);
OneNnBound one_nn_bound(const GridDev &g, double search_radius);
int one_nn_warm_reserve(dcreg_ctx *c);
struct OneNnLaunch {
    PoseArg P; OneNnBound bound;
    bool dump;
    const uint32_t *warm_in; uint32_t *warm_out;
    double *partials; uint32_t nb;
};
int one_nn_run(dcreg_ctx *c, const double *R, const double *t, const dcreg_lin_params *p, dcreg_lin_out *out, const char *what,
               int (*extra)(dcreg_ctx *, const dcreg_ctx::FrameSet *fs), const std::function<void(const OneNnLaunch &)> &launch, bool dump,
               const DumpField *fields, int n_fields);
int rows_batch_check(dcreg_ctx *c, int slot, int n_poses, const double *R9, const double *t3, const dcreg_lin_params *p, bool ids_given, const char *what,
                     bool search);
int rows_batch_clouds(dcreg_ctx *c, const dcreg_ctx::FrameSet *fs, int n_poses, const int32_t *ids, const char *noun,
// ... 123 lines not shown
```

dcreg_amd/csrc/device/kernels.hpp:

```cpp
#pragma once
#include <hip/hip_runtime.h>
#include <stdint.h>
#include <type_traits>

#include "search.hpp"

namespace dcreg {

template <int CTRL, int ROW_MASK>
__device__ __forceinline__ double dpp_add(double v) {
    const uint64_t b = (uint64_t)__double_as_longlong(v);
    int lo = (int)(uint32_t)b, hi = (int)(uint32_t)(b >> 32);
    lo = __builtin_amdgcn_update_dpp(0, lo, CTRL, ROW_MASK, 0xF, ROW_MASK == 0xF);
    hi = __builtin_amdgcn_update_dpp(0, hi, CTRL, ROW_MASK, 0xF, ROW_MASK == 0xF);
    const double o = __longlong_as_double((long long)(((uint64_t)(uint32_t)hi << 32) | (uint32_t)lo));
    return v + o;
}
__device__ __forceinline__ double wave_sum_to_lane63(double v) {
    v = dpp_add<0x111, 0xF>(v);
    v = dpp_add<0x112, 0xF>(v);
    v = dpp_add<0x114, 0xF>(v);
    v = dpp_add<0x118, 0xF>(v);
    v = dpp_add<0x142, 0xA>(v);
    v = dpp_add<0x143, 0xC>(v);
// ... 263 lines not shown
                    if (lane <= 9) gt.pose_out->R[lane - 1] = d; else gt.pose_out->t[lane - 10] = d;
                }
                if (lane == 0) { gt.pose_out->state = 0; gt.pose_out->fresh = gt.fresh; *gt.abort_out = call_off ? 1u : 0u; }
            }
            if (lane < kGateWords) __hip_atomic_store(&gd->w[lane], hv, __ATOMIC_RELAXED, __HIP_MEMORY_SCOPE_AGENT);
        }
        for (;;) {
            whole = gate_read<__HIP_MEMORY_SCOPE_AGENT>(gd->w, v, seq);
            if (whole && (seq >> 1) == gt.want) break;
            __builtin_amdgcn_s_sleep(8);
        }
    }
    if ((seq & 1ull) != 0ull) return false;
#pragma unroll
    for (int k = 0; k < 12; ++k) {
        const uint32_t lo = (uint32_t)__builtin_amdgcn_readlane((int)(uint32_t)v, k + 1), hi = (uint32_t)__builtin_amdgcn_readlane((int)(uint32_t)(v >> 32), k + 1);
        const double d = __longlong_as_double((long long)(((unsigned long long)hi << 32) | lo));
        if (k < 9) P.R[k] = d; else P.t[k - 9] = d;
    }
    return true;
}

__device__ __forceinline__ void wave_rows_to_lds(const double (&row)[8], uint8_t flag, double *stage, double *gm, double (*cnt)[2],
                                                 double extra0 = 0.0, double extra1 = 0.0) {
    const int lane = threadIdx.x & 63, wave = threadIdx.x >> 6;
    double u0, u1;
    wave_gram_mfma(row, stage, lane, u0, u1);
    if ((lane & 15) < 8) {
        gm[(lane >> 4) * 8 + (lane & 7)] = u0;
        gm[32 + (lane >> 4) * 8 + (lane & 7)] = u1;
    }
    const unsigned long long eff = __builtin_amdgcn_ballot_w64(flag == 1), inr = __builtin_amdgcn_ballot_w64(flag != 0);
    if (lane == 0) { cnt[wave][0] = (double)__builtin_popcountll(eff) + extra0; cnt[wave][1] = (double)__builtin_popcountll(inr) + extra1; }
}
__device__ __forceinline__ double block_slot_sum(const double *gm0, int gm_stride, const double (*cnt)[2]) {
    double t = 0.0;
    if (threadIdx.x < 29) {
        const int e = gram_entry_of_slot(threadIdx.x);
#pragma unroll
        for (int w = 0; w < kLinBlock / 64; ++w) t += gm0[w * gm_stride + e];
    } else if (threadIdx.x < 31) {
#pragma unroll
        for (int w = 0; w < kLinBlock / 64; ++w) t += cnt[w][threadIdx.x - 29];
    }
    return t;
}
template <bool FUSED>
__device__ __forceinline__ void block_publish(const double *gm0, int gm_stride, double (*red)[kSlots], double (*cnt)[2], int *s_role, double *my_rows, uint32_t vb,
                                              uint32_t n_blocks_x, const FinArgs &fin, uint32_t pose_id) {
    if (threadIdx.x < kSlots) {
        const double t = block_slot_sum(gm0, gm_stride, cnt);
        if (FUSED && fin.direct) {
            publish_row(fin.out + (size_t)vb * kSlots, t, fin.seq);
        } else if (FUSED) {
            st_agent(my_rows + (size_t)vb * kSlots + threadIdx.x, t);
            wait_stores();
        } else {
            my_rows[(size_t)vb * kSlots + threadIdx.x] = t;
        }
    }
    if (FUSED && !fin.direct) {
        const uint32_t chunk = vb / kChunk;
        const uint32_t csize = min((uint32_t)kChunk, n_blocks_x - chunk * kChunk);
        const size_t gchunk = (size_t)pose_id * fin.chunks_per_pose + chunk;
        __syncthreads();
        if (threadIdx.x == 0) {
            const unsigned int prev = __hip_atomic_fetch_add(&fin.tickets[gchunk * kCounterStride], 1u, __ATOMIC_RELAXED, __HIP_MEMORY_SCOPE_AGENT);
            *s_role = (prev == csize - 1) ? 1 : 0;
            if (prev == csize - 1) __hip_atomic_store(&fin.tickets[gchunk * kCounterStride], 0u, __ATOMIC_RELAXED, __HIP_MEMORY_SCOPE_AGENT);
        }
        __syncthreads();
        if (*s_role == 1) {
            const double t = block_sum_rows(my_rows + (size_t)chunk * kChunk * kSlots, csize, red);
            double *orow = fin.out + gchunk * kSlots;
            if (threadIdx.x < 32) publish_row(orow, t, fin.seq);
        }
    }
}

constexpr int kLinDepth = 2;
constexpr int kAdvTile = 1536;
static_assert(kAdvTile % kLinBlock == 0 && kAdvTile <= 65536, "a tile is a whole number of query blocks; list entries are 16-bit offsets");

template <int MODE, bool FUSED, bool FAST, bool GATE = false, bool ONE = false, bool SLICE = false, bool GRIDS = false>
static __global__ __launch_bounds__(ONE ? kWave : kLinBlock, kLinOcc) void k_lin(const float4 *__restrict__ src, uint32_t n_src, GridDev g,
                                                          PoseArg pose1, const PoseArg *__restrict__ poses, LinArgs a,
                                                          double *__restrict__ partials, uint32_t n_blocks_x, FinArgs fin,
                                                          DebugDev dbg, const uint32_t *__restrict__ abort_flag, GateArgs gt,
                                                          const uint2 *__restrict__ slices, const PairGrid *__restrict__ grids,
                                                          const uint32_t *__restrict__ grid_ids) {
    if (abort_flag && *abort_flag != 0u) return;
    static_assert(!ONE || (MODE == 0 && FUSED && !GATE), "the one-wave instantiation is the fused product launch behind k_gate");
    static_assert(!SLICE || (MODE == 0 && !GATE), "per-pose source slices are batched product launches");
    static_assert(!GRIDS || SLICE, "per-pose target grids come with per-pose source slices");
    if constexpr (GRIDS) {
        const PairGrid &pg = grids[grid_ids[blockIdx.y]];
        g = pg.g; a.max_ring = pg.max_ring; a.infl_max_d2 = pg.infl_max_d2;
    }
    constexpr int kWavesHere = ONE ? 1 : kLinBlock / kWave;
    __shared__ double red[ONE ? 1 : kLinBlock / 32][kSlots];
    __shared__ double cnt[kWavesHere][2];
    __shared__ int s_role;
    __shared__ RunList runs[kWavesHere];
    static_assert(sizeof(RunList) >= sizeof(double) * (kWave * kRowStride + 64), "the one-wave block's reduction lives in its RunList");
    const double *const gm0 = &red[0][0];
    constexpr int gm_stride = 64;
    const int wave = threadIdx.x >> 6;
    const uint32_t pose_id = blockIdx.y;
    const uint32_t vbt = ONE ? xcd_remap(blockIdx.x, n_blocks_x * (kLinBlock / kWave), a.xcd_chunk * (kLinBlock / kWave)) : 0u;
    uint32_t vb = ONE ? vbt / (kLinBlock / kWave) : xcd_remap(blockIdx.x, n_blocks_x, a.xcd_chunk);
    const uint32_t tile = ONE ? vbt % (kLinBlock / kWave) : (uint32_t)wave;
    if (!GRIDS && a.n_groups) {
        const uint32_t lead = n_blocks_x - a.n_groups * a.group_blocks;
        if (vb >= lead) {
            const uint32_t slot = (vb - lead) / a.group_blocks;
            vb = lead + (uint32_t)a.group_order[slot] * a.group_blocks + (vb - lead) % a.group_blocks;
        }
    }
    uint32_t nb_pose = n_blocks_x;
    if constexpr (SLICE) {
        const uint2 sl = slices[blockIdx.y];
        nb_pose = (sl.y + kLinBlock - 1) / kLinBlock;
        if (vb >= nb_pose) return;
        src += sl.x; n_src = sl.y;
    }
    const uint32_t i = ONE ? vb * kLinBlock + tile * kWave + threadIdx.x : vb * kLinBlock + threadIdx.x;
    auto stamp = [&](int k, unsigned long long v) {
        if constexpr (MODE == 2) {
            if ((threadIdx.x & 63) == 0 && dbg.stamps) dbg.stamps[((size_t)vb * (kLinBlock / 64) + wave) * 8 + k] = v;
        }
    };
    if constexpr (MODE == 2) stamp(0, __builtin_readcyclecounter());
    PoseArg P;
    if (poses) P = poses[pose_id]; else P = pose1;
    uint8_t flag = 0;
    const bool have_q = i < n_src;
    const bool keep = a.state != nullptr && P.state != kNoIdx;
    const bool old = keep && P.fresh == 0u;
    const bool CERT = old && a.use_cert != 0;
    uint32_t *const sbase = keep ? a.state + (size_t)P.state * kStateRows * a.state_stride : nullptr;
    const size_t ss = a.state_stride;
    typedef double dbl2 __attribute__((ext_vector_type(2)));
    uint4 *const SV0 = reinterpret_cast<uint4 *>(sbase + kStV0 * ss), *const SX = reinterpret_cast<uint4 *>(sbase + kStX * ss);
    dbl2 *const SV1 = reinterpret_cast<dbl2 *>(sbase + kStV1 * ss), *const SV2 = reinterpret_cast<dbl2 *>(sbase + kStV2 * ss);
    uint32_t *const SW3 = sbase + kStW3 * ss;
    uint2 *const SY = reinterpret_cast<uint2 *>(sbase + kStY * ss);
    const float4 s4 = have_q ? src[i] : make_float4(0.f, 0.f, 0.f, 0.f);
    uint32_t cert = kCertSearch, fitw = kFitNone, q0[3] = {0u, 0u, 0u};
    dbl2 p01 = {0.0, 0.0}, p23 = {0.0, 0.0};
    if (CERT && have_q) {
        const uint4 v0 = SV0[i];
        p01 = SV1[i]; p23 = SV2[i];
        cert = v0.x; fitw = v0.y; q0[0] = v0.z; q0[1] = v0.w; q0[2] = SW3[i];
    }
    if constexpr (GATE) {
        unsigned long long gate_v = 0ull, gate_seq = 0ull;
        const bool gate_whole = gate_read<__HIP_MEMORY_SCOPE_AGENT>(gt.dev->w, gate_v, gate_seq);
        if (!gate_wait(gt, gate_v, gate_seq, gate_whole, P)) return;
    }
    float qx, qy, qz;
    body_to_global(P, (double)s4.x, (double)s4.y, (double)s4.z, qx, qy, qz);
    const float q0x = __uint_as_float(q0[0]), q0y = __uint_as_float(q0[1]), q0z = __uint_as_float(q0[2]);
    const bool need = have_q && !(CERT && cert_holds(cert, q0x, q0y, q0z, qx, qy, qz));
    bool refit = have_q && !need && !cert_is_out(cert) && !fit_holds(fitw, q0x, q0y, q0z, qx, qy, qz);
    uint32_t stats = 0;
    uint32_t w_search = 0, w_refit = 0;
    uint32_t adv_s = 0, adv_r = 0;
    if (a.adv_counts && tile == 0u) {
        adv_s = a.adv_counts[(size_t)vb * kCounterStride]; adv_r = a.adv_counts[(size_t)vb * kCounterStride + 1];
        if ((threadIdx.x & 63u) == 0u) { a.adv_counts[(size_t)vb * kCounterStride] = 0u; a.adv_counts[(size_t)vb * kCounterStride + 1] = 0u; }
    }
    KnnResult<5> nn;
    Fit fit;
    uint8_t gate = 255;
    const bool level3 = have_q && !need && !refit && !cert_is_out(cert);
    auto stored_plane = [&](const dbl2 &a01, const dbl2 &a23) {
        gate = (uint8_t)(fitw & 3u);
        fit.plane[0] = a01.x; fit.plane[1] = a01.y; fit.plane[2] = a23.x; fit.plane[3] = a23.y;
    };
    if constexpr (MODE == 2) { asm volatile("s_waitcnt vmcnt(0)" ::: "memory"); stamp(1, __builtin_readcyclecounter()); }
    if (!wave_any(need || refit)) {
        if (level3) stored_plane(p01, p23);
    } else {
        uint32_t pos6[6];
#pragma unroll
        for (int j = 0; j < 6; ++j) pos6[j] = kNoIdx;
        uint32_t iw = i;
        asm volatile("" : "+v"(iw));
        const unsigned long long need_mask = __builtin_amdgcn_ballot_w64(need);
        w_search = (uint32_t)__builtin_popcountll(need_mask);
        if (need_mask != 0ull) {
            if (a.search_count && (threadIdx.x & 63) == 0)
                atomicAdd(a.search_count + (size_t)(blockIdx.x & 63u) * (kCounterStride / 2), (unsigned long long)__builtin_popcountll(need_mask));
            const bool warm = old && a.warm != 0;
            if (warm && need) {
                const uint4 x = SX[i];
                const uint2 y = SY[i];
                pos6[0] = x.x; pos6[1] = x.y; pos6[2] = x.z; pos6[3] = x.w; pos6[4] = y.x; pos6[5] = y.y;
            }
            bool by_team = false;
            if (warm && w_search <= (uint32_t)a.team_max) {
                float tb = 0.f;
                bool tight = false;
                if (need && pos6[5] != kNoIdx) tb = team_bound(g, a, pos6, qx, qy, qz, tight);
                if (!wave_any(need && !tight)) {
                    uint32_t tpos[6], tcert;
                    by_team = team_search6(g, runs[wave].team, a, need_mask, qx, qy, qz, tb, tpos, tcert) == need_mask;
                    if (a.search_count && by_team && (threadIdx.x & 63) == 0)
                        atomicAdd(a.search_count + (size_t)(blockIdx.x & 63u) * (kCounterStride / 2) + 1, (unsigned long long)w_search);
                    if (by_team && need) {
                        cert = tcert;
#pragma unroll
                        for (int j = 0; j < 6; ++j) pos6[j] = tpos[j];
                    }
                }
            }
            if (!by_team) {
                Set6 s6;
                uint32_t c2;
                lin_search6<kLinSweep, kLinDepth>(g, runs[wave], a, need, warm, pos6, qx, qy, qz, s6, c2);
                if (need) {
                    cert = c2;
#pragma unroll
                    for (int j = 0; j < 6; ++j) pos6[j] = s6.pos[j];
                    stats = (s6.n_eval & 0xFFFFu) | ((s6.n_shell & 0x7FFFu) << 16);
                }
            }
            if (need && keep) {
                SX[iw] = make_uint4(pos6[0], pos6[1], pos6[2], pos6[3]);
                SY[iw] = make_uint2(pos6[4], pos6[5]);
            }
        }
        if constexpr (MODE == 2) { asm volatile("s_waitcnt vmcnt(0)" ::: "memory"); stamp(2, __builtin_readcyclecounter()); stamp(6, (unsigned long long)w_search); }
        const bool set = have_q && !cert_is_out(cert);
        const bool fitnow = set && (need || refit);
        w_refit = (uint32_t)__builtin_popcountll(__builtin_amdgcn_ballot_w64(fitnow && !need));
        if (wave_any(fitnow)) {
            const bool use6 = fitnow && cert_is_set6(cert);
            const bool six = wave_any(use6);
            const bool presorted = !wave_any(fitnow && !need);
            if (fitnow && !need) {
                const uint4 x = SX[iw];
                const uint2 y = SY[iw];
                pos6[0] = x.x; pos6[1] = x.y; pos6[2] = x.z; pos6[3] = x.w; pos6[4] = y.x; pos6[5] = y.y;
            }
            if (!use6) pos6[5] = kNoIdx;
            if (fitnow) {
                const uint8_t in_r = fit_from_set<FAST>(g, a, qx, qy, qz, pos6, six, nn, fit, presorted);
                gate = in_r ? (uint8_t)(fit.word & 3u) : (uint8_t)255;
                if (keep) {
                    if (!need) {
                        const uint4 o0 = SV0[iw];
                        const uint32_t o1 = SW3[iw];
                        cert = cert_rebased(cert, __uint_as_float(o0.z), __uint_as_float(o0.w), __uint_as_float(o1), qx, qy, qz);
                    }
                    SV0[iw] = make_uint4(cert, fit.word, __float_as_uint(qx), __float_as_uint(qy));
                    SV1[iw] = dbl2{fit.plane[0], fit.plane[1]};
                    SV2[iw] = dbl2{fit.plane[2], fit.plane[3]};
                    SW3[iw] = __float_as_uint(qz);
                }
            }
        }
        if constexpr (MODE == 2) { asm volatile("s_waitcnt vmcnt(0)" ::: "memory"); stamp(3, __builtin_readcyclecounter()); stamp(7, (unsigned long long)w_refit); }
        if (level3) {
            const dbl2 b01 = SV1[iw], b23 = SV2[iw];
            fitw = reinterpret_cast<const uint32_t *>(SV0 + iw)[1];
            stored_plane(b01, b23);
        }
        if (!set && need && keep) {
            SV0[iw] = make_uint4(cert, kFitNone, __float_as_uint(qx), __float_as_uint(qy));
            SW3[iw] = __float_as_uint(qz);
        }
    }
    double nrm[3] = {0.0, 0.0, 0.0}, r_pt = 0.0, s_pt = 0.0;
    double row[8];
#pragma unroll
    for (int k = 0; k < 8; ++k) row[k] = 0.0;
    if (have_q) {
        if (gate == 0) flag = row_of_plane<FAST>(P, a, s4, qx, qy, qz, fit.plane, row, nrm, r_pt, s_pt);
        else flag = gate == 255 ? (uint8_t)0 : gate;
    }
    if constexpr (MODE == 2) stamp(4, __builtin_readcyclecounter());
    if (MODE == 1 && have_q) {
        const uint32_t oi = __float_as_uint(s4.w);
#pragma unroll
        for (int j = 0; j < 5; ++j) {
            if (dbg.nn_idx) dbg.nn_idx[5 * (size_t)oi + j] = flag != 0 ? (int32_t)nn.idx[j] : -1;
            if (dbg.nn_d2) dbg.nn_d2[5 * (size_t)oi + j] = flag != 0 ? nn.d2[j] : __builtin_inff();
        }
        if (flag == 1 || flag == 4) {
            if (dbg.normal) { dbg.normal[3 * (size_t)oi] = nrm[0]; dbg.normal[3 * (size_t)oi + 1] = nrm[1]; dbg.normal[3 * (size_t)oi + 2] = nrm[2]; }
            if (dbg.r) dbg.r[oi] = r_pt;
            if (dbg.s) dbg.s[oi] = s_pt;
        }
        if (dbg.flag) dbg.flag[oi] = flag;
        if (dbg.stats) dbg.stats[oi] = stats;
    }
    if constexpr (ONE) {
        double *const gm = runs[0].stage + kWave * kRowStride;
        wave_rows_to_lds(row, flag, runs[0].stage, gm, cnt, a.count_scale * (double)(w_search + adv_s), a.count_scale * (double)(w_refit + adv_r));
        __syncthreads();
        constexpr uint32_t T = kLinBlock / kWave;
        if (threadIdx.x < kSlots) {
            double t = 0.0;
            if (threadIdx.x < 29) t = gm[gram_entry_of_slot(threadIdx.x)];
            else if (threadIdx.x < 31) t = cnt[0][threadIdx.x - 29];
            partials[(((size_t)pose_id * n_blocks_x + vb) * T + tile) * kSlots + threadIdx.x] = t;
        }
    } else {
    wave_rows_to_lds(row, flag, runs[wave].stage, &red[0][0] + wave * gm_stride, cnt, a.count_scale * (double)(w_search + adv_s),
                     a.count_scale * (double)(w_refit + adv_r));
    if constexpr (MODE == 2) stamp(5, __builtin_readcyclecounter());
    __syncthreads();
    block_publish<FUSED>(gm0, gm_stride, red, cnt, &s_role, partials + (size_t)pose_id * n_blocks_x * kSlots, vb, nb_pose, fin, pose_id);
    }
}

constexpr int kAdvDepth = 4;
constexpr int kAdvRowsBatch = 6;
static_assert((kAdvTile / kLinBlock) % kAdvRowsBatch == 0 && kAdvTile / kLinBlock <= kChunk, "whole batches; a tile spans at most two chunks");
template <bool FAST, bool ROWS = false>
static __global__ __launch_bounds__(kLinBlock, (kAdvDepth > 2 ? 2 : kLinOcc)) void k_advance(const float4 *__restrict__ src, uint32_t n_src, GridDev g, PoseArg pose1,
                                                                              const PoseArg *__restrict__ poses, LinArgs a,
                                                                              uint32_t *__restrict__ counts, const uint32_t *__restrict__ abort_flag,
                                                                              double *__restrict__ partials, uint32_t n_blocks_x, FinArgs fin) {
    if (abort_flag && *abort_flag != 0u) return;
    __shared__ RunList runs[kLinBlock / kWave];
    __shared__ uint16_t list[kAdvTile];
    __shared__ uint32_t n_list[2];
    __shared__ double red[kLinBlock / 32][kSlots];
    __shared__ double cnt[ROWS ? kAdvTile / kLinBlock : 1][kLinBlock / kWave][2];
    static_assert(sizeof(RunList) >= sizeof(double) * (kWave * kRowStride + (kAdvTile / kLinBlock) * 64), "a wave's Gram matrices of a tile live in its RunList");
    __shared__ uint32_t nofit[kAdvTile / 32];
    __shared__ int s_role;
    const int lane = threadIdx.x & 63, wave = threadIdx.x >> 6;
    PoseArg P;
    if (poses) P = poses[0]; else P = pose1;
    const size_t ss = a.state_stride;
    uint32_t *const sbase = a.state + (size_t)P.state * kStateRows * ss;
    typedef double dbl2 __attribute__((ext_vector_type(2)));
    uint4 *const SV0 = reinterpret_cast<uint4 *>(sbase + kStV0 * ss), *const SX = reinterpret_cast<uint4 *>(sbase + kStX * ss);
    dbl2 *const SV1 = reinterpret_cast<dbl2 *>(sbase + kStV1 * ss), *const SV2 = reinterpret_cast<dbl2 *>(sbase + kStV2 * ss);
    uint32_t *const SW3 = sbase + kStW3 * ss;
    uint2 *const SY = reinterpret_cast<uint2 *>(sbase + kStY * ss);
    if (threadIdx.x < 2) n_list[threadIdx.x] = 0u;
    if constexpr (ROWS) { if (threadIdx.x < (uint32_t)(kAdvTile / 32)) nofit[threadIdx.x] = 0u; }
    __syncthreads();
    const uint32_t base = blockIdx.x * (uint32_t)kAdvTile;
    constexpr int U = kAdvTile / kLinBlock;
    {
        float4 s4[U];
        uint4 v0[U];
        uint32_t w3[U];
#pragma unroll
// ... 1193 lines not shown
```

dcreg_amd/csrc/device/search.hpp:

```cpp
#pragma once
#include <stddef.h>
#include <stdint.h>
#if defined(DCREG_HOST_EMUL)
#define DCREG_DEVFN inline
#define DCREG_ON_DEVICE 0
#else
#include <hip/hip_runtime.h>
#if defined(__HIP_DEVICE_COMPILE__) && !defined(__gfx950__)
#error "these kernels are written for gfx950 (CDNA4): inline ISA, wave64 DPP, sc1 coherence protocol"
#endif
#define DCREG_DEVFN __device__ __forceinline__
#define DCREG_ON_DEVICE 1
#endif

namespace dcreg {

#if DCREG_ON_DEVICE
DCREG_DEVFN float med3f(float a, float b, float c) { return __builtin_amdgcn_fmed3f(a, b, c); }
#define DCREG_STAT(field) ((void)0)
#define DCREG_TRACE(kk, dz, dy, which, trips) ((void)0)
#else
inline float med3f(float a, float b, float c) { return fmaxf(fminf(a, b), fminf(fmaxf(a, b), c)); }
#define DCREG_STAT(field) (++emu_stats.field)
#define DCREG_TRACE(kk, dz, dy, which, trips) emu_trace_push(((((uint32_t)(kk) << 20) | ((uint32_t)((dz) + 512) << 10) | (uint32_t)((dy) + 512)) << 1) | (uint32_t)(which), (uint32_t)(trips))
#endif

constexpr int kBlock = 256;
constexpr int kLinOcc = 4;
constexpr int kLinBlock = 256;
constexpr int kSlots = 32;
constexpr uint32_t kNoIdx = 0xFFFFFFFFu;

struct GridDev {
    double ox, oy, oz;
    double inv_h, h;
    int nx, ny, nz;
    int sx;
    uint32_t n_pts;
    const uint32_t *cell_start;
    const float4 *pts;
    const uint8_t *gap;
    int gap_cap;
    const uint32_t *owner;
    const uint32_t *ymask;
    int nxb, nyw;
};

struct PoseArg {
    double R[9]; double t[3];
    uint32_t state;
    uint32_t fresh;
};
constexpr int kStateRows = 19;
constexpr uint32_t kCertSearch = 0xFFFFFFFFu;
constexpr int kStV0 = 0, kStV1 = 4, kStV2 = 8, kStW3 = 12, kStX = 13, kStY = 17;
DCREG_DEVFN size_t state_word_index(int row, size_t i, size_t S) {
    constexpr uint8_t grp[19] = {13, 13, 13, 13, 17, 17,  0, 0, 0, 12, 0, 4, 4, 4, 4, 8, 8, 8, 8};
    constexpr uint8_t wpe[19] = { 4,  4,  4,  4,  2,  2,  4, 4, 4,  1, 4, 4, 4, 4, 4, 4, 4, 4, 4};
    constexpr uint8_t sub[19] = { 0,  1,  2,  3,  0,  1,  0, 2, 3,  0, 1, 0, 1, 2, 3, 0, 1, 2, 3};
    return (size_t)grp[row] * S + i * wpe[row] + sub[row];
}

struct LinArgs {
    double radius_sq;
    float radius_sq_f;
    float cert_r_out;
    float cert_r_in;
    double max_thick_sq, min_norm, w_slope, w_min;
    int use_wd;
    int max_ring;
    int warm;
    int use_cert;
    int team_max;
    float prune_infl;
    float infl_max_d2;
    unsigned long long *search_count;
    uint32_t *state;
    uint32_t state_stride;
    uint32_t group_blocks, n_groups;
    uint8_t group_order[256];
    uint32_t xcd_chunk;
    double count_scale;
    uint32_t *adv_counts;
    float far_loose;
    int euler;
// ... 77 lines not shown
                "v_cndmask_b32_e64 %[p4], %[p4], %[p3], %[m3]\n\t"
                "v_cndmask_b32_e64 %[p3], %[p3], %[p], %[m3]\n\t"
                "v_cndmask_b32_e64 %[p3], %[p3], %[p2], %[m2]\n\t"
                "v_cndmask_b32_e64 %[p2], %[p2], %[p], %[m2]\n\t"
                "v_cndmask_b32_e64 %[p2], %[p2], %[p1], %[m1]\n\t"
                "v_cndmask_b32_e64 %[p1], %[p1], %[p], %[m1]\n\t"
                "v_cndmask_b32_e64 %[p1], %[p1], %[p0], %[m0]\n\t"
                "v_cndmask_b32_e64 %[p0], %[p0], %[p], %[m0]"
                : [d0] "+v"(d[0]), [d1] "+v"(d[1]), [d2] "+v"(d[2]), [d3] "+v"(d[3]), [d4] "+v"(d[4]),
                  [p0] "+v"(pos[0]), [p1] "+v"(pos[1]), [p2] "+v"(pos[2]), [p3] "+v"(pos[3]), [p4] "+v"(pos[4]),
                  [om] "+v"(outside_min), [t] "=&v"(t),
                  [m0] "=&s"(m0), [m1] "=&s"(m1), [m2] "=&s"(m2), [m3] "=&s"(m3), [m4] "=&s"(m4)
                : [x] "v"(d2), [p] "v"(p));
        } else if constexpr (K == 6) {
            unsigned long long m0, m1, m2, m3, m4, m5;
            float t;
            asm("v_cmp_lt_f32_e64 %[m0], %[x], %[d0]\n\t"
                "v_cmp_lt_f32_e64 %[m1], %[x], %[d1]\n\t"
                "v_cmp_lt_f32_e64 %[m2], %[x], %[d2]\n\t"
                "v_cmp_lt_f32_e64 %[m3], %[x], %[d3]\n\t"
                "v_cmp_lt_f32_e64 %[m4], %[x], %[d4]\n\t"
                "v_cmp_lt_f32_e64 %[m5], %[x], %[d5]\n\t"
                "v_max_f32_e32 %[t], %[x], %[d5]\n\t"
                "v_min_f32_e32 %[om], %[om], %[t]\n\t"
                "v_med3_f32 %[d5], %[d4], %[d5], %[x]\n\t"
                "v_med3_f32 %[d4], %[d3], %[d4], %[x]\n\t"
                "v_med3_f32 %[d3], %[d2], %[d3], %[x]\n\t"
                "v_med3_f32 %[d2], %[d1], %[d2], %[x]\n\t"
                "v_med3_f32 %[d1], %[d0], %[d1], %[x]\n\t"
                "v_min_f32_e32 %[d0], %[d0], %[x]\n\t"
                "v_cndmask_b32_e64 %[p5], %[p5], %[p], %[m5]\n\t"
                "v_cndmask_b32_e64 %[p5], %[p5], %[p4], %[m4]\n\t"
                "v_cndmask_b32_e64 %[p4], %[p4], %[p], %[m4]\n\t"
                "v_cndmask_b32_e64 %[p4], %[p4], %[p3], %[m3]\n\t"
                "v_cndmask_b32_e64 %[p3], %[p3], %[p], %[m3]\n\t"
                "v_cndmask_b32_e64 %[p3], %[p3], %[p2], %[m2]\n\t"
                "v_cndmask_b32_e64 %[p2], %[p2], %[p], %[m2]\n\t"
                "v_cndmask_b32_e64 %[p2], %[p2], %[p1], %[m1]\n\t"
                "v_cndmask_b32_e64 %[p1], %[p1], %[p], %[m1]\n\t"
                "v_cndmask_b32_e64 %[p1], %[p1], %[p0], %[m0]\n\t"
                "v_cndmask_b32_e64 %[p0], %[p0], %[p], %[m0]"
                : [d0] "+v"(d[0]), [d1] "+v"(d[1]), [d2] "+v"(d[2]), [d3] "+v"(d[3]), [d4] "+v"(d[4]), [d5] "+v"(d[5]),
                  [p0] "+v"(pos[0]), [p1] "+v"(pos[1]), [p2] "+v"(pos[2]), [p3] "+v"(pos[3]), [p4] "+v"(pos[4]), [p5] "+v"(pos[5]),
                  [om] "+v"(outside_min), [t] "=&v"(t),
                  [m0] "=&s"(m0), [m1] "=&s"(m1), [m2] "=&s"(m2), [m3] "=&s"(m3), [m4] "=&s"(m4), [m5] "=&s"(m5)
                : [x] "v"(d2), [p] "v"(p));
        } else
#endif
        {
            outside_min = fminf(outside_min, fmaxf(d2, d[K - 1]));
            bool c[K];
#pragma unroll
            for (int i = 0; i < K; ++i) c[i] = d2 < d[i];
#pragma unroll
            for (int i = K - 1; i >= 1; --i) {
                pos[i] = c[i - 1] ? pos[i - 1] : (c[i] ? p : pos[i]);
                d[i] = med3f(d[i - 1], d[i], d2);
            }
            pos[0] = c[0] ? p : pos[0];
            d[0] = fminf(d[0], d2);
        }
    }
    DCREG_DEVFN float worst_d2() const { return fmaxf(d[K - 1], fminf(d[K - 1] * infl, cap)); }
    DCREG_DEVFN float dist(int j) const { return d[j]; }
    DCREG_DEVFN bool full() const { return pos[K - 1] != kNoIdx; }
    DCREG_DEVFN bool boundary_tie() const { return full() && outside_min == d[K - 1]; }
};

struct Top6 {
    static constexpr int K = 6;
    float d[6];
    uint32_t n_eval, n_shell;
    DCREG_DEVFN void init(float bound_f) {
#pragma unroll
        for (int i = 0; i < 6; ++i) d[i] = bound_f;
        n_eval = 0; n_shell = 1;
    }
    DCREG_DEVFN void push(float x, uint32_t , uint32_t , bool  = true) {
        d[5] = med3f(d[4], d[5], x); d[4] = med3f(d[3], d[4], x); d[3] = med3f(d[2], d[3], x);
        d[2] = med3f(d[1], d[2], x); d[1] = med3f(d[0], d[1], x); d[0] = fminf(d[0], x);
    }
};

DCREG_DEVFN float dist2_nofma(float qx, float qy, float qz, const float4 &c) {
#pragma clang fp contract(off)
    typedef float f2 __attribute__((ext_vector_type(2)));
    f2 dxy = f2{qx, qy} - f2{c.x, c.y};
    dxy = dxy * dxy;
    const float dz = qz - c.z;
    float d2 = dxy.x + dxy.y;
    d2 = d2 + dz * dz;
    return d2;
}

DCREG_DEVFN void body_to_global(const PoseArg &P, double px, double py, double pz, float &qx, float &qy, float &qz) {
#pragma clang fp contract(off)
    qx = (float)(P.R[0] * px + P.R[1] * py + P.R[2] * pz + P.t[0]);
    qy = (float)(P.R[3] * px + P.R[4] * py + P.R[5] * pz + P.t[1]);
    qz = (float)(P.R[6] * px + P.R[7] * py + P.R[8] * pz + P.t[2]);
}

template <class H, int NB = 1>
DCREG_DEVFN void scan_run(const GridDev &g, uint32_t s, uint32_t e, float qx, float qy, float qz, H &hp);

DCREG_DEVFN int clampi(int v, int lo, int hi) { return min(max(v, lo), hi); }
DCREG_DEVFN float sqrt_approx(float x) {
#if DCREG_ON_DEVICE
    return __builtin_amdgcn_sqrtf(x);
#else
    return sqrtf(x);
#endif
}

struct RunList;
template <class H, bool SWEEP, bool NOTE>
DCREG_DEVFN void knn_shells(const GridDev &g, RunList &rl, float qx, float qy, float qz, int cx, int cy, int cz,
                                           double fx, double fy, double fz, float bound_f, int max_ring, H &hp);

constexpr int kPend = 7;
static_assert(kPend >= 4, "a trip parks up to four candidates: the pending list must hold them");
constexpr int kWave = 64;
struct PendEntry { uint32_t d2_bits, pos; };
constexpr int kRowStride = 9;
struct TeamLds { uint32_t d2[kWave], pos[kWave], idx[kWave]; uint32_t out_d2[8], out_pos[8]; };
struct alignas(16) RunList {
    union {
        struct {
            uint32_t s[9][kWave];
            uint32_t e[9][kWave];
            uint16_t gap2h[9][kWave];
            PendEntry pend[kPend][kWave];
        };
        double stage[kWave * kRowStride];
        TeamLds team;
    };
};
DCREG_DEVFN bool wave_any(bool x) {
#if DCREG_ON_DEVICE
    return __builtin_amdgcn_ballot_w64(x) != 0ull;
#else
    return x;
#endif
}

template <class H>
DCREG_DEVFN void push_point(H &hp, float qx, float qy, float qz, const float4 &c, uint32_t p, bool valid) {
    const float d2 = dist2_nofma(qx, qy, qz, c);
    hp.push(valid ? d2 : __builtin_inff(), __float_as_uint(c.w), p, valid);
}

constexpr int kPtsPad = 16;
constexpr int kProbeBatch = 2;
template <class H, int NB>
DCREG_DEVFN void scan_run(const GridDev &g, uint32_t s, uint32_t e, float qx, float qy, float qz, H &hp) {
    static_assert(4 * NB <= kPtsPad, "slots past the end of the array read its padding");
    DCREG_STAT(runs);
    for (uint32_t p = s; p < e; p += 4 * NB) {
        float4 c[4 * NB];
        const float4 *cp4 = g.pts + p;
#pragma unroll
        for (int u = 0; u < 4 * NB; ++u) c[u] = cp4[u];
#pragma unroll
        for (int u = 0; u < 4 * NB; ++u) {
            if (u % 4 == 0 && p + u < e) DCREG_STAT(trips);
            push_point<H>(hp, qx, qy, qz, c[u], p + u, p + u < e);
        }
    }
}

template <class H, bool NOTE>
DCREG_DEVFN void scan_run_deferred(const GridDev &g, RunList &rl, uint32_t s, uint32_t e, float qx, float qy, float qz, H &hp) {
    DCREG_STAT(runs);
    const int tid = threadIdx.x & (kWave - 1);
    float lim = hp.worst_d2();
    float om = __builtin_inff();
    int cnt = 0;
    auto flush = [&]() {
        for (int j = 0; j < cnt; ++j) {
            const PendEntry pe = rl.pend[j][tid];
            hp.template push<false>(__uint_as_float(pe.d2_bits), 0u, pe.pos, true);
        }
        cnt = 0;
        lim = hp.worst_d2();
    };
    auto take4 = [&](const float4 (&c)[4], uint32_t p) {
        DCREG_STAT(trips);
        if (wave_any(cnt > kPend - 4)) flush();
#pragma unroll
        for (int u = 0; u < 4; ++u) {
            const float d2 = dist2_nofma(qx, qy, qz, c[u]);
            const bool valid = p + u < e;
            const bool pass = valid && d2 < lim;
            hp.n_eval += valid ? 1u : 0u;
            if (pass) { rl.pend[cnt][tid] = PendEntry{__float_as_uint(d2), p + u}; ++cnt; }
            if (NOTE) om = fminf(om, (valid && !pass) ? d2 : __builtin_inff());
        }
    };
    auto load4 = [&](float4 (&c)[4], uint32_t p) {
        const float4 *cp4 = g.pts + p;
#pragma unroll
        for (int u = 0; u < 4; ++u) c[u] = cp4[u];
    };
    float4 ca[4], cb[4];
    if (s < e) load4(ca, s);
    for (uint32_t p = s; p < e; p += 8) {
        const bool second = p + 4 < e;
        if (second) load4(cb, p + 4);
        take4(ca, p);
        if (!second) break;
        if (p + 8 < e) load4(ca, p + 8);
        take4(cb, p + 4);
    }
    flush();
    if (NOTE) hp.note_outside(om);
}

template <class H, bool SWEEP = false, bool NOTE = true, int DEPTH = 2>
DCREG_DEVFN void knn_search(const GridDev &g, RunList &rl, float qx, float qy, float qz, float bound_f,
                                           int max_ring, H &hp, float infl = 1.f, float cap = __builtin_inff(), bool empty_block = false) {
    hp.init(bound_f, infl, cap);
    const double fx = ((double)qx - g.ox) * g.inv_h, fy = ((double)qy - g.oy) * g.inv_h, fz = ((double)qz - g.oz) * g.inv_h;
    const double lim = (double)max_ring + 1.0;
    if (max_ring >= 0) {
        if (fx < -lim || fy < -lim || fz < -lim || fx > g.nx + lim || fy > g.ny + lim || fz > g.nz + lim) return;
    }
    const double big = 6.0e7;
    const double flx = floor(fmin(fmax(fx, -big), big)), fly = floor(fmin(fmax(fy, -big), big)), flz = floor(fmin(fmax(fz, -big), big));
    const int cx = (int)flx, cy = (int)fly, cz = (int)flz;
    const int nx = g.nx, ny = g.ny, nz = g.nz;
    if (max_ring < 0) {
        const int ex = max(abs(cx), abs(cx - (nx - 1))), ey = max(abs(cy), abs(cy - (ny - 1))), ez = max(abs(cz), abs(cz - (nz - 1)));
        max_ring = max(ex, max(ey, ez)) + 1;
    }

    const int tid = threadIdx.x & (kWave - 1);
    int nrun = 0;
    if (!empty_block) {
        const float hf = (float)g.h;
        const float frx = (float)(fx - flx), fry = (float)(fy - fly), frz = (float)(fz - flz);
        const float gyl = fry * hf, gyh = (1.f - fry) * hf, gzl = frz * hf, gzh = (1.f - frz) * hf;
        const float gy2[3] = {gyl * gyl * 0.99999f, 0.f, gyh * gyh * 0.99999f}, gz2[3] = {gzl * gzl * 0.99999f, 0.f, gzh * gzh * 0.99999f};
        const int sx = g.sx, nxf = nx * sx;
        const int cxs = cx * sx;
        const float uf = frx * (float)sx;
        const float kx = (float)g.inv_h * (float)sx * 1.00001f;
        const uint32_t unx = (uint32_t)nxf, uny = (uint32_t)ny, sxy = unx * uny;
        const uint32_t base_c = ((uint32_t)cz * uny + (uint32_t)cy) * unx;
        const uint32_t yoff[3] = {base_c - unx, base_c, base_c + unx};
        const bool yok[3] = {(uint32_t)(cy - 1) < uny, (uint32_t)cy < uny, (uint32_t)(cy + 1) < uny};
        const bool zok[3] = {(uint32_t)(cz - 1) < (uint32_t)nz, (uint32_t)cz < (uint32_t)nz, (uint32_t)(cz + 1) < (uint32_t)nz};
        constexpr int DY[9] = {0, -1, 1, 0, 0, -1, 1, -1, 1};
        constexpr int DZ[9] = {0, 0, 0, -1, 1, -1, -1, 1, 1};
        uint32_t rs[9], re[9];
        float g2s[9];
#pragma unroll
        for (int r = 0; r < 9; ++r) {
            const float g2 = gy2[DY[r] + 1] + gz2[DZ[r] + 1];
            g2s[r] = g2;
            const float rxf = fminf(sqrt_approx(fmaxf(bound_f - g2, 0.f)) * kx + 1e-4f, 1.0e6f);
            const int lo = max((int)floorf(uf - rxf), -sx), hi = min((int)floorf(uf + rxf), 2 * sx - 1);
            const int x0 = clampi(cxs + lo, 0, nxf), x1 = clampi(cxs + hi + 1, 0, nxf);
            const bool ok = yok[DY[r] + 1] && zok[DZ[r] + 1] && (x1 > x0) && !(g2 > bound_f);
            const uint32_t row = yoff[DY[r] + 1] + (DZ[r] < 0 ? 0u - sxy : (DZ[r] > 0 ? sxy : 0u));
            rs[r] = g.cell_start[ok ? row + (uint32_t)x0 : 0u];
            re[r] = g.cell_start[ok ? row + (uint32_t)x1 : 0u];
            if (ok) { DCREG_STAT(table_loads); DCREG_STAT(table_loads); }
        }
#pragma unroll
        for (int r = 0; r < 9; ++r) {
            if (re[r] > rs[r]) {
                rl.s[nrun][tid] = rs[r]; rl.e[nrun][tid] = re[r]; rl.gap2h[nrun][tid] = (uint16_t)(__float_as_uint(g2s[r]) >> 16);
                ++nrun;
            }
        }
    }
    if (!empty_block) {
        int ri = 0;
        uint32_t p = 0, e = 0;
        float lim = bound_f, om = __builtin_inff();
        int cnt = 0;
        auto next_run = [&]() {
            const float g2 = __uint_as_float((uint32_t)rl.gap2h[ri][tid] << 16);
            const uint32_t s_ = rl.s[ri][tid], e_ = rl.e[ri][tid];
            ++ri;
            const bool keep = !(g2 > (H::kDeferred ? lim : hp.worst_d2()));
            p = keep ? s_ : 0u; e = keep ? e_ : 0u;
            DCREG_STAT(runs);
        };
        constexpr int W = 4;
        struct Slot { float4 c[W]; uint32_t cp, ce; bool live; };
        bool have = nrun > 0;
        if (have) next_run();
        auto fetch = [&](Slot &sl) {
            sl.live = have; sl.cp = p; sl.ce = e;
            if (have) {
                DCREG_STAT(trips);
                const float4 *cp4 = g.pts + p;
#pragma unroll
                for (int u = 0; u < W; ++u) sl.c[u] = cp4[u];
                p += W;
                if (p >= e) {
                    have = ri < nrun;
                    if (have) next_run();
                }
            }
        };
        auto flush = [&]() {
            if constexpr (H::kDeferred) {
                for (int j = 0; j < cnt; ++j) {
                    const PendEntry pe = rl.pend[j][tid];
                    hp.template push<false>(__uint_as_float(pe.d2_bits), 0u, pe.pos, true);
                }
                cnt = 0;
                lim = hp.worst_d2();
            }
        };
        auto consume = [&](const Slot &sl) {
            if constexpr (H::kDeferred) {
#pragma unroll
                for (int u = 0; u < W; ++u) {
                    const float d2 = dist2_nofma(qx, qy, qz, sl.c[u]);
                    const bool valid = sl.cp + u < sl.ce;
                    const bool pass = valid && d2 < lim;
                    hp.n_eval += valid ? 1u : 0u;
                    if (pass) { rl.pend[cnt][tid] = PendEntry{__float_as_uint(d2), sl.cp + u}; ++cnt; }
                    if (NOTE) om = fminf(om, (valid && !pass) ? d2 : __builtin_inff());
                }
            } else {
#pragma unroll
                for (int u = 0; u < W; ++u) push_point<H>(hp, qx, qy, qz, sl.c[u], sl.cp + u, sl.cp + u < sl.ce);
            }
        };
        Slot S[DEPTH];
#pragma unroll
        for (int k = 0; k < DEPTH - 1; ++k) fetch(S[k]);
        bool go = DEPTH > 1 ? S[0].live : have;
        while (go) {
#pragma unroll
            for (int k = 0; k < DEPTH; ++k) {
                if (H::kDeferred && wave_any(cnt > kPend - W)) flush();
                fetch(S[(k + DEPTH - 1) % DEPTH]); consume(S[k]);
                if (!S[(k + 1) % DEPTH].live) { go = false; break; }
            }
        }
        if constexpr (H::kDeferred) {
            flush();
            hp.note_outside(om);
        }
    }
    knn_shells<H, SWEEP, NOTE>(g, rl, qx, qy, qz, cx, cy, cz, fx, fy, fz, bound_f, max_ring, hp);
}

template <class H, bool SWEEP, bool NOTE>
DCREG_DEVFN void knn_shells(const GridDev &g, RunList &rl, float qx, float qy, float qz, int cx, int cy, int cz,
                                           double fx, double fy, double fz, float bound_f, int max_ring, H &hp) {
    const int nx = g.nx, ny = g.ny, nz = g.nz;
    const float hf = (float)g.h;
    bool done;
    {
        const double safe = g.h * (1.0 - 1e-9);
        const double safe2 = safe * safe * (1.0 - 1e-6);
        done = max_ring <= 1 || (double)hp.worst_d2() <= safe2 || safe2 >= (double)bound_f;
        if (!wave_any(!done)) return;
    }
    int k0 = 1;
    if (!SWEEP && g.gap && cx >= 0 && cx < nx && cy >= 0 && cy < ny && cz >= 0 && cz < nz) {
        const int f = min((int)g.gap[((int64_t)cz * ny + cy) * nx + cx], g.gap_cap + 1);
        k0 = max(1, f - 1);
    }
    auto lookup_scan = [&](int64_t c0, int64_t c1) {
        DCREG_STAT(table_loads); DCREG_STAT(table_loads); DCREG_STAT(faces);
        const uint32_t s_ = g.cell_start[c0], e_ = g.cell_start[c1];
        if constexpr (SWEEP && H::kDeferred) scan_run_deferred<H, NOTE>(g, rl, s_, e_, qx, qy, qz, hp);
        else scan_run<H>(g, s_, e_, qx, qy, qz, hp);
    };
    const float frx = (float)(fx - (double)cx), fry = (float)(fy - (double)cy), frz = (float)(fz - (double)cz);
    const float inv_hf = (float)g.inv_h;
    const int sx = g.sx, nxf = nx * sx;
    const int cxs = cx * sx;
    const float uf = frx * (float)sx, inv_hfs = inv_hf * (float)sx;
    auto slab = [&](int c, int cq, float fr) -> float {
        return c < cq ? ((float)(cq - c - 1) + fr) * hf : (c > cq ? ((float)(c - cq) - fr) * hf : 0.f);
    };
    auto face_row = [&](int y, int z, float dyz, int kk, int dz, int dy) {
        DCREG_STAT(rows);
        const float w = hp.worst_d2();
        if (dyz > w) return;
        const float xr_c = fminf((sqrt_approx(w - dyz) * 1.00001f) * inv_hfs + 1e-4f, 1.0e6f);
        const int dlo = (int)floorf(uf - xr_c), dhi = (int)floorf(uf + xr_c);
        const int kks = min(kk, 1 << 26) * sx;
        const int x0 = max(cxs + max(dlo, -kks), 0), x1 = min(cxs + min(dhi, kks + sx - 1), nxf - 1) + 1;
        if (x1 <= x0) return;
        const int64_t row = ((int64_t)z * ny + y) * nxf;
        DCREG_TRACE(kk, dz, dy, 0, (g.cell_start[row + x1] - g.cell_start[row + x0] + 3u) / 4u);
        lookup_scan(row + x0, row + x1);
    };
    auto reach = [&](float r2, float fr, int cap, int &lo, int &hi) {
        const float rc = fminf(sqrt_approx(fmaxf(r2, 0.f)) * 1.00001f * inv_hf + 1e-4f, 1.0e6f);
        lo = -min(cap, (int)floorf(rc + 1.f - fr));
        hi = min(cap, (int)floorf(rc + fr));
        if (r2 < 0.f) { lo = 1; hi = 0; }
    };
    if constexpr (SWEEP) {
        const float w0 = hp.worst_d2();
        if (!done) {
            const int nxb = g.nxb, nyw = g.nyw, cap = 1 << 24;
            auto sweep_row = [&](int y, int z, float gz) {
                DCREG_STAT(rows);
                const float gy = slab(y, cy, fry);
                const float dyz = (gy * gy + gz * gz) * 0.99999f;
                const float w = hp.worst_d2();
                if (dyz > w) return;
                const float xr_c = fminf((sqrt_approx(w - dyz) * 1.00001f) * inv_hfs + 1e-4f, 1.0e6f);
                const int dlo = (int)floorf(uf - xr_c), dhi = (int)floorf(uf + xr_c);
                const int x0 = max(cxs + dlo, 0), x1 = min(cxs + dhi, nxf - 1) + 1;
                if (x1 <= x0) return;
                const int64_t row = ((int64_t)z * ny + y) * nxf;
                if (abs(y - cy) <= 1 && abs(z - cz) <= 1) {
                    const int l1 = min(x1, cxs - sx), r0 = max(x0, cxs + 2 * sx);
                    if (l1 > x0) lookup_scan(row + x0, row + l1);
                    if (x1 > r0) lookup_scan(row + r0, row + x1);
                } else {
                    lookup_scan(row + x0, row + x1);
                }
            };
            int zlo, zhi;
            reach(w0, frz, cap, zlo, zhi);
            const int zmax = max(-zlo, zhi);
            for (int i = 0; i <= 2 * zmax; ++i) {
                const int adz = (i + 1) >> 1, dz = (i & 1) ? -adz : adz;
                const float w = hp.worst_d2();
                { const float nearer = (float)max(adz - 1, 0) * hf; if (nearer * nearer * 0.99999f > w) break; }
                const int z = cz + dz;
                if (z < 0 || z >= nz) continue;
                const float gz = slab(z, cz, frz);
                const float rem = w - gz * gz * 0.99999f;
                if (rem < 0.f) continue;
                int ylo, yhi, xlo, xhi;
                reach(rem, fry, cap, ylo, yhi);
                reach(rem, frx, cap, xlo, xhi);
                const int y0 = max(cy + ylo, 0), y1 = min(cy + yhi, ny - 1);
                const int b0 = max(cx + xlo, 0) >> 4, b1 = min(cx + xhi, nx - 1) >> 4;
                if (y1 < y0 || b1 < b0) continue;
                for (int yw = y0 >> 5; yw <= (y1 >> 5); ++yw) {
                    uint32_t m = 0;
                    const uint32_t *mw = g.ymask + ((int64_t)z * nxb + b0) * nyw + yw;
                    for (int b = b0; b <= b1; ++b, mw += nyw) { m |= *mw; DCREG_STAT(table_loads); }
                    const int lo = max(y0 - (yw << 5), 0), hi = min(y1 - (yw << 5), 31);
                    m &= (0xFFFFFFFFu >> (31 - hi)) & (0xFFFFFFFFu << lo);
                    while (m) {
                        const int bit = __builtin_ctz(m);
                        m &= m - 1;
                        sweep_row((yw << 5) + bit, z, gz);
                    }
                }
            }
// ... 357 lines not shown
    {
        n1 = 0.0; n2 = 0.0;
#pragma unroll
        for (int i = 1; i < 5; ++i) { n1 += c1[i] * c1[i]; n2 += c2[i] * c2[i]; }
        const bool b2 = n2 > n1;
        const double big = b2 ? n2 : n1;
        if (nz == 3 && big < thr_helper * 4.0) nz = 1;
        swap_col(c1, c2, b2); swap_i(p1, p2, b2);
        householder_fast<1>(c0, c1, c2, uk, coef, rdiag, rinv);
    }
    {
        n2 = 0.0;
#pragma unroll
        for (int i = 2; i < 5; ++i) n2 += c2[i] * c2[i];
        if (nz == 3 && n2 < thr_helper * 3.0) nz = 2;
        householder_fast<2>(c0, c1, c2, uk, coef, rdiag, rinv);
    }
    double c[5] = {-1.0, -1.0, -1.0, -1.0, -1.0};
    if (nz > 0) {
        double w = uk[0] * c[0];
#pragma unroll
        for (int i = 1; i < 5; ++i) w += c0[i] * c[i];
        w *= coef[0];
        c[0] -= w * uk[0];
#pragma unroll
        for (int i = 1; i < 5; ++i) c[i] -= w * c0[i];
    }
    if (nz > 1) {
        double w = uk[1] * c[1];
#pragma unroll
        for (int i = 2; i < 5; ++i) w += c1[i] * c[i];
        w *= coef[1];
        c[1] -= w * uk[1];
#pragma unroll
        for (int i = 2; i < 5; ++i) c[i] -= w * c1[i];
    }
    if (nz > 2) {
        double w = uk[2] * c[2];
#pragma unroll
        for (int i = 3; i < 5; ++i) w += c2[i] * c[i];
        w *= coef[2];
        c[2] -= w * uk[2];
    }
    double y0 = 0.0, y1 = 0.0, y2 = 0.0;
    if (nz > 2) y2 = c[2] * rinv[2];
    if (nz > 1) y1 = (c[1] - (nz > 2 ? c2[1] * y2 : 0.0)) * rinv[1];
    if (nz > 0) y0 = (c[0] - (nz > 1 ? c1[0] * y1 : 0.0) - (nz > 2 ? c2[0] * y2 : 0.0)) * rinv[0];
    x[0] = (p0 == 0) ? y0 : ((p1 == 0) ? y1 : y2);
    x[1] = (p0 == 1) ? y0 : ((p1 == 1) ? y1 : y2);
    x[2] = (p0 == 2) ? y0 : ((p1 == 2) ? y1 : y2);
}

struct PointQuery {
    float qx, qy, qz;
    bool reach;
};

struct Set6 {
    uint32_t pos[6];
    float d2[6];
    float lb7;
    uint32_t n_eval, n_shell;
};

template <bool SWEEP, int DEPTH = 2>
DCREG_DEVFN void search6(const GridDev &g, RunList &rl, float qx, float qy, float qz, float bound_f, int max_ring, float infl, float cap, Set6 &out,
                         bool empty_block = false) {
    HeapFast<6> hf;
    knn_search<HeapFast<6>, SWEEP, false, DEPTH>(g, rl, qx, qy, qz, bound_f, max_ring, hf, infl, cap, empty_block);
    out.n_eval = hf.n_eval; out.n_shell = hf.n_shell;
#pragma unroll
    for (int j = 0; j < 6; ++j) { out.pos[j] = hf.pos[j]; out.d2[j] = hf.d[j]; }
    out.lb7 = fminf(hf.outside_min, fminf(hf.worst_d2(), bound_f));
    if (hf.pos[5] != kNoIdx && hf.d[4] == hf.d[5]) {
        HeapExact<6> he;
        knn_search<HeapExact<6>, SWEEP>(g, rl, qx, qy, qz, bound_f, max_ring, he, 1.f, __builtin_inff(), empty_block);
        out.n_eval += he.n_eval;
#pragma unroll
        for (int j = 0; j < 6; ++j) { out.pos[j] = he.pos[j]; out.d2[j] = he.dist(j); }
        out.lb7 = out.d2[5];
    }
}

DCREG_DEVFN uint32_t make_cert(const Set6 &s, const LinArgs &a) {
    const float a4 = sqrt_approx(s.d2[4]), a5 = sqrt_approx(s.d2[5]), a6 = sqrt_approx(s.lb7);
    const float s_out = a4 * 0.999998f - a.cert_r_out;
    const float s5 = s.pos[4] != kNoIdx ? 0.5f * (a5 * 0.999998f - a4 * 1.000002f) : -1.f;
    const float s6 = s.pos[5] != kNoIdx ? 0.5f * (a6 * 0.999998f - a4 * 1.000002f) : -1.f;
    if (s_out > 0.f && s_out >= fmaxf(s5, s6)) return __float_as_uint(s_out) | 0x80000000u;
    if (s6 > s5) return (__float_as_uint(fmaxf(s6 * 0.9999998f, 0.f)) & ~1u) | 1u;
    return __float_as_uint(fmaxf(s5, 0.f)) & ~1u;
}
DCREG_DEVFN bool cert_is_out(uint32_t cert) { return (cert & 0x80000000u) != 0u; }
DCREG_DEVFN bool cert_is_set6(uint32_t cert) { return (cert & 0x80000001u) == 1u; }

DCREG_DEVFN bool cert_holds(uint32_t cert, float q0x, float q0y, float q0z, float qx, float qy, float qz) {
    const float dx = qx - q0x, dy = qy - q0y, dz = qz - q0z;
    const float m2 = (dx * dx + dy * dy + dz * dz) * 1.00001f;
    const float s = __uint_as_float(cert & 0x7FFFFFFFu);
    return m2 < s * s;
}

DCREG_DEVFN float warm_bound6(const GridDev &g, const uint32_t (&oldpos)[6], float qx, float qy, float qz, float bound) {
    float4 pv[6];
#pragma unroll
    for (int j = 0; j < 6; ++j) pv[j] = g.pts[oldpos[j]];
    float m = 0.f;
#pragma unroll
    for (int j = 0; j < 6; ++j) m = fmaxf(m, dist2_nofma(qx, qy, qz, pv[j]));
    const float incl = fmaxf(__uint_as_float(__float_as_uint(m) + 1u), 1.17549435e-38f);
    return fminf(bound, incl);
}

template <bool SWEEP, int DEPTH = 2>
DCREG_DEVFN void lin_search6(const GridDev &g, RunList &runs, const LinArgs &a, bool have_q, bool warm, const uint32_t (&oldpos)[6],
                             float qx, float qy, float qz, Set6 &st, uint32_t &cert) {
    float bound = a.radius_sq_f;
    if (warm && oldpos[5] != kNoIdx) bound = warm_bound6(g, oldpos, qx, qy, qz, bound);
    const double fx = ((double)qx - g.ox) * g.inv_h, fy = ((double)qy - g.oy) * g.inv_h, fz = ((double)qz - g.oz) * g.inv_h;
    const double lim = (double)a.max_ring + 1.0;
    const bool reach = have_q && !(fx < -lim || fy < -lim || fz < -lim || fx > g.nx + lim || fy > g.ny + lim || fz > g.nz + lim);
    bool all_in_space = false;
    if (g.owner) {
        bool far = false;
        uint32_t oc = kNoIdx;
        bool in_space = false;
        const float loose0 = a.far_loose * (float)g.h;
        const bool maybe = reach && bound > loose0 * loose0;
        if (wave_any(maybe)) {
            if (maybe) {
                const int ix = clampi((int)floor(fx), 0, g.nx - 1), iy = clampi((int)floor(fy), 0, g.ny - 1), iz = clampi((int)floor(fz), 0, g.nz - 1);
                const double outd = fmax(fmax(fmax(-fx, fx - (double)g.nx), fmax(-fy, fy - (double)g.ny)), fmax(fmax(-fz, fz - (double)g.nz), 0.0));
                const int out = (int)ceil(fmin(outd, 1.0e6));
                const int64_t cell = ((int64_t)iz * g.ny + iy) * g.nx + ix;
                const int f0 = (int)g.gap[cell];
                const int f = f0 + out;
                in_space = f >= 2 && (out == 0 || out >= 2);
                const float loose = ((float)f + a.far_loose) * (float)g.h;
                if (f0 != 255 && (bound > loose * loose || bound >= a.radius_sq_f)) { oc = g.owner[cell]; far = oc != kNoIdx; }
            }
            all_in_space = !wave_any(reach && !in_space);
        }
        if (wave_any(far)) {
            Top6 hb;
            hb.init(bound);
            uint32_t s_ = 0, e_ = 0;
            if (far) {
                const uint32_t ox = oc % (uint32_t)g.nx;
                const uint32_t row = (oc - ox) * (uint32_t)g.sx;
                s_ = g.cell_start[row + (ox > 0u ? ox - 1u : 0u) * (uint32_t)g.sx];
                e_ = g.cell_start[row + min(ox + 2u, (uint32_t)g.nx) * (uint32_t)g.sx];
                e_ = min(e_, s_ + 48u);
            }
            scan_run<decltype(hb), kProbeBatch>(g, s_, e_, qx, qy, qz, hb);
            bool more = far && e_ - s_ < 6u && !(hb.d[5] < bound);
            if (wave_any(more)) {
                uint32_t ox = 0, oy = 0, oz = 0;
                if (more) { ox = oc % (uint32_t)g.nx; const uint32_t r_ = oc / (uint32_t)g.nx; oy = r_ % (uint32_t)g.ny; oz = r_ / (uint32_t)g.ny; }
#pragma unroll 1
                for (int k = 0; k < 4 && wave_any(more); ++k) {
                    uint32_t s2 = 0, e2 = 0;
                    if (more) {
                        const int yy = (int)oy + (k == 0 ? -1 : (k == 1 ? 1 : 0)), zz = (int)oz + (k == 2 ? -1 : (k == 3 ? 1 : 0));
                        if (yy >= 0 && yy < g.ny && zz >= 0 && zz < g.nz) {
                            const uint32_t row2 = ((uint32_t)zz * (uint32_t)g.ny + (uint32_t)yy) * (uint32_t)g.nx * (uint32_t)g.sx;
                            s2 = g.cell_start[row2 + (ox > 0u ? ox - 1u : 0u) * (uint32_t)g.sx];
                            e2 = g.cell_start[row2 + min(ox + 2u, (uint32_t)g.nx) * (uint32_t)g.sx];
                            e2 = min(e2, s2 + 48u);
                        }
                    }
                    scan_run<decltype(hb), kProbeBatch>(g, s2, e2, qx, qy, qz, hb);
                    more = far && !(hb.d[5] < bound);
                }
            }
            if (far) bound = fminf(bound, fmaxf(__uint_as_float(__float_as_uint(hb.d[5]) + 1u), 1.17549435e-38f));
        }
    }
    const float infl = a.prune_infl, cap = a.infl_max_d2 * a.prune_infl;
    bound = fminf(fmaxf(bound, fminf(bound * infl, cap)), a.radius_sq_f);
#pragma unroll
    for (int j = 0; j < 6; ++j) { st.pos[j] = kNoIdx; st.d2[j] = bound; }
    st.lb7 = bound; st.n_eval = 0; st.n_shell = 1;
    if (reach) search6<SWEEP, DEPTH>(g, runs, qx, qy, qz, bound, a.max_ring, infl, cap, st, SWEEP && all_in_space);
    cert = make_cert(st, a);
}


DCREG_DEVFN void team_row(const GridDev &g, float qx, float qy, float qz, float bound_f, int dy, int dz, uint32_t &s_out, uint32_t &e_out) {
    const double fx = ((double)qx - g.ox) * g.inv_h, fy = ((double)qy - g.oy) * g.inv_h, fz = ((double)qz - g.oz) * g.inv_h;
    const double big = 6.0e7;
    const double flx = floor(fmin(fmax(fx, -big), big)), fly = floor(fmin(fmax(fy, -big), big)), flz = floor(fmin(fmax(fz, -big), big));
    const int cx = (int)flx, cy = (int)fly, cz = (int)flz;
    const int nx = g.nx, ny = g.ny, nz = g.nz;
    const float hf = (float)g.h;
    const float frx = (float)(fx - flx), fry = (float)(fy - fly), frz = (float)(fz - flz);
    const float gyl = fry * hf, gyh = (1.f - fry) * hf, gzl = frz * hf, gzh = (1.f - frz) * hf;
    const float gy2 = dy < 0 ? gyl * gyl * 0.99999f : (dy > 0 ? gyh * gyh * 0.99999f : 0.f);
    const float gz2 = dz < 0 ? gzl * gzl * 0.99999f : (dz > 0 ? gzh * gzh * 0.99999f : 0.f);
    const int sx = g.sx, nxf = nx * sx;
    const int cxs = cx * sx;
    const float uf = frx * (float)sx;
    const float kx = (float)g.inv_h * (float)sx * 1.00001f;
    const uint32_t unx = (uint32_t)nxf, uny = (uint32_t)ny, sxy = unx * uny;
    const bool yok = (uint32_t)(cy + dy) < uny, zok = (uint32_t)(cz + dz) < (uint32_t)nz;
    const float g2 = gy2 + gz2;
    const float rxf = fminf(sqrt_approx(fmaxf(bound_f - g2, 0.f)) * kx + 1e-4f, 1.0e6f);
    const int lo = max((int)floorf(uf - rxf), -sx), hi = min((int)floorf(uf + rxf), 2 * sx - 1);
    const int x0 = clampi(cxs + lo, 0, nxf), x1 = clampi(cxs + hi + 1, 0, nxf);
    const bool ok = yok && zok && (x1 > x0) && !(g2 > bound_f);
    const uint32_t row = ((uint32_t)(cz + dz) * uny + (uint32_t)(cy + dy)) * unx;
    (void)sxy;
    s_out = g.cell_start[ok ? row + (uint32_t)x0 : 0u];
    e_out = g.cell_start[ok ? row + (uint32_t)x1 : 0u];
}

struct BallCells { int cx, cy, cz; float frx, fry, frz; int ylo, yhi, zlo, zhi; };
DCREG_DEVFN BallCells ball_cells(const GridDev &g, float qx, float qy, float qz, float bound_f) {
    const double fx = ((double)qx - g.ox) * g.inv_h, fy = ((double)qy - g.oy) * g.inv_h, fz = ((double)qz - g.oz) * g.inv_h;
    const double big = 6.0e7;
    const double flx = floor(fmin(fmax(fx, -big), big)), fly = floor(fmin(fmax(fy, -big), big)), flz = floor(fmin(fmax(fz, -big), big));
    BallCells b;
    b.cx = (int)flx; b.cy = (int)fly; b.cz = (int)flz;
    b.frx = (float)(fx - flx); b.fry = (float)(fy - fly); b.frz = (float)(fz - flz);
    const float rc = fminf(sqrt_approx(fmaxf(bound_f, 0.f)) * 1.00001f * (float)g.inv_h + 1e-4f, 1.0e6f);
    const int cap = 1 << 24;
    b.ylo = -min(cap, (int)floorf(rc + 1.f - b.fry)); b.yhi = min(cap, (int)floorf(rc + b.fry));
    b.zlo = -min(cap, (int)floorf(rc + 1.f - b.frz)); b.zhi = min(cap, (int)floorf(rc + b.frz));
    return b;
}
DCREG_DEVFN void ball_row(const GridDev &g, const BallCells &b, float bound_f, int dy, int dz, uint32_t &s_out, uint32_t &e_out) {
    const float hf = (float)g.h;
    const float gy = dy < 0 ? ((float)(-dy - 1) + b.fry) * hf : (dy > 0 ? ((float)dy - b.fry) * hf : 0.f);
    const float gz = dz < 0 ? ((float)(-dz - 1) + b.frz) * hf : (dz > 0 ? ((float)dz - b.frz) * hf : 0.f);
    const float dyz = (gy * gy + gz * gz) * 0.99999f;
    const int sx = g.sx, nxf = g.nx * sx;
    const int cxs = b.cx * sx;
    const float uf = b.frx * (float)sx, inv_hfs = (float)g.inv_h * (float)sx;
    const float xr_c = fminf((sqrt_approx(fmaxf(bound_f - dyz, 0.f)) * 1.00001f) * inv_hfs + 1e-4f, 1.0e6f);
    const int dlo = (int)floorf(uf - xr_c), dhi = (int)floorf(uf + xr_c);
    const int x0 = max(cxs + dlo, 0), x1 = min(cxs + dhi, nxf - 1) + 1;
    const int y = b.cy + dy, z = b.cz + dz;
    const bool ok = !(dyz > bound_f) && y >= 0 && y < g.ny && z >= 0 && z < g.nz && x1 > x0;
    const uint32_t row = ((uint32_t)z * (uint32_t)g.ny + (uint32_t)y) * (uint32_t)nxf;
    s_out = g.cell_start[ok ? row + (uint32_t)x0 : 0u];
    e_out = g.cell_start[ok ? row + (uint32_t)x1 : 0u];
}

DCREG_DEVFN float team_bound(const GridDev &g, const LinArgs &a, const uint32_t (&oldpos)[6], float qx, float qy, float qz, bool &tight) {
    float bound = warm_bound6(g, oldpos, qx, qy, qz, a.radius_sq_f);
    const float infl = a.prune_infl, cap = a.infl_max_d2 * a.prune_infl;
    bound = fminf(fmaxf(bound, fminf(bound * infl, cap)), a.radius_sq_f);
    const double fx = ((double)qx - g.ox) * g.inv_h, fy = ((double)qy - g.oy) * g.inv_h, fz = ((double)qz - g.oz) * g.inv_h;
    const double lim = (double)a.max_ring + 1.0;
    const bool reach = !(fx < -lim || fy < -lim || fz < -lim || fx > g.nx + lim || fy > g.ny + lim || fz > g.nz + lim);
    const double safe = g.h * (1.0 - 1e-9);
    tight = reach && (double)bound <= safe * safe * (1.0 - 1e-6);
    return bound;
}

#if DCREG_ON_DEVICE
constexpr int kTeamPre = 4;
constexpr int kTeamMax = 7;
DCREG_DEVFN float readlane_f(float v, int l) { return __uint_as_float((uint32_t)__builtin_amdgcn_readlane((int)__float_as_uint(v), l)); }
DCREG_DEVFN uint32_t readlane_u(uint32_t v, int l) { return (uint32_t)__builtin_amdgcn_readlane((int)v, l); }
DCREG_DEVFN float shfl_f(float v, int src) { return __uint_as_float((uint32_t)__builtin_amdgcn_ds_bpermute(src << 2, (int)__float_as_uint(v))); }

DCREG_DEVFN unsigned long long team_search6(const GridDev &g, TeamLds &T, const LinArgs &a, unsigned long long team_mask, float qx, float qy,
// ... 363 lines not shown
```

Measured before the change: 16730.

## Add five-neighbour search mode for large-step ICP linearisations

Adds a 'five' linearisation path that, when the pose step is large and most points need a search anyway, runs a plain 5-NN search instead of the 6-NN search with certificates, team passes and refit bookkeeping. The host plan chooses this mode from the last step size and the searched fraction, and tracks state_five/five_tail so later launches re-search points whose warm state came from five-neighbour results. It also generalises the starting-bound probe to K neighbours and lets warm bounds work from five stored neighbours. The aim is to cut per-point search and certificate overhead during early, large-motion iterations, at the cost of more plan complexity and lost certificate reuse right after a five launch.

```diff
diff --git a/dcreg_amd/api.py b/dcreg_amd/api.py
--- a/dcreg_amd/api.py
+++ b/dcreg_amd/api.py
@@ -2346,7 +2346,7 @@
         if hasattr(self._L, "dcreg_launch_series_structure"):
             self._L.dcreg_launch_series_structure(self._h, st.ctypes.data_as(C.POINTER(C.c_uint8)), n)
         self._L.dcreg_launch_series(self._h, _dp(ms), se.ctypes.data_as(lp), rf.ctypes.data_as(lp), pt.ctypes.data_as(lp), n, int(reset))
-        return {"ms": ms, "searched": se, "refitted": rf, "points": pt, "advanced": adv & 3, "one_wave": (adv >> 2) & 1, "structure": st}
+        return {"ms": ms, "searched": se, "refitted": rf, "points": pt, "advanced": adv & 3, "one_wave": (adv >> 2) & 1, "structure": st & 3, "five": (st >> 2) & 1}
 
     def team_pass_stamps(self):
         n = self._L.dcreg_team_pass_stamps(self._h, None, 0)
diff --git a/dcreg_amd/csrc/device/context.hip b/dcreg_amd/csrc/device/context.hip
--- a/dcreg_amd/csrc/device/context.hip
+++ b/dcreg_amd/csrc/device/context.hip
@@ -1425,6 +1425,7 @@
     const uint2 *d_slices;
     const uint32_t *d_grid_ids;
     bool state_was_valid;
+    bool state_was_five;
     bool own() const { return kind >= LinKind::single; }
     bool uses_state(const dcreg_ctx *c) const { return own() && c->opt_warm; }
 };
@@ -1510,12 +1511,14 @@
     const double f = known ? (double)c->last_searched / (double)L.n : -1.0;
     if ((L.kind == LinKind::single || L.kind == LinKind::gated) && c->opt_warm && !fresh && P.use_cert && L.a.count_scale != 0.0) {
         constexpr double kAdvanceLo = 0.005, kAdvanceHi = 0.70;
-        const bool adv = c->opt_advance >= 2 || (c->opt_advance == 1 && P.nbx >= (uint32_t)c->opt_advance_min_blocks && known && f >= kAdvanceLo && f <= kAdvanceHi);
+        const bool in_window = (known && f >= kAdvanceLo && f <= kAdvanceHi) || c->five_tail > 0;
+        const bool adv = c->opt_advance >= 2 || (c->opt_advance == 1 && P.nbx >= (uint32_t)c->opt_advance_min_blocks && in_window);
         constexpr double kTeamPassMaxPoints = 16384.0, kTeamPassMinFrac = 0.5, kTeamPassMinCellPts = 3.0;
         const double per_cell = (double)c->map.n / (double)std::max<uint32_t>(c->map.occupied, 1u);
         const bool team = c->opt_team_pass >= 2 || (c->opt_team_pass == 1 && L.n <= (int64_t)kTeamPassMaxPoints && known && f >= kTeamPassMinFrac &&
                                                     per_cell >= kTeamPassMinCellPts);
         P.pass = team ? LinPass::team : adv ? LinPass::advance : LinPass::none;
+        if (c->opt_search_five >= 2 && c->opt_advance < 2 && c->opt_team_pass < 2) P.pass = LinPass::none;
     }
     bool one_wave = false;
     if (L.n_poses > 1)
@@ -1529,6 +1532,11 @@
     P.body = (P.gate_inside && P.pass != LinPass::team) ? LinBody::gated : L.kind == LinKind::stamps ? LinBody::stamps : L.kind == LinKind::dump ? LinBody::dump :
              one_wave ? LinBody::one_wave : fused ? LinBody::fused : LinBody::chunked;
     P.pass_rows = P.pass == LinPass::advance && c->opt_advance_fused != 0 && !P.direct && P.body == LinBody::fused;
+    const bool can_five = (L.kind == LinKind::single || L.kind == LinKind::gated) && L.uses_state(c) && !dbg && P.pass == LinPass::none &&
+                          (P.body == LinBody::fused || P.body == LinBody::one_wave);
+    P.five = can_five && (c->opt_search_five >= 2 ||
+                          (c->opt_search_five == 1 && P.use_cert && (fresh || (known && f >= c->opt_search_five_frac)) &&
+                           c->last_step > c->opt_search_five_step * c->map.grid.h));
     return P;
 }
 
@@ -1645,7 +1653,7 @@
         if (dbg->stamps) dd.stamps = (unsigned long long *)alloc(sizeof(unsigned long long) * 8 * (kLinBlock / 64) * (size_t)P.nbx, 0);
         if (oom) { free_tmp(S); drop_warm(c); c->fail("hipMalloc of the debug dump buffers failed"); return DCREG_E_NOMEM; }
     }
-    L.a.use_cert = P.use_cert ? 1 : 0;
+    L.a.use_cert = (P.use_cert && !(P.five && c->state_five && L.state_was_valid)) ? 1 : 0;
     L.a.search_count = c->opt_count_searches ? c->d_search_count.data() : nullptr;
     L.a.group_blocks = std::max<uint32_t>(c->group_blocks, 1u); L.a.n_groups = P.ordered ? c->n_groups : 0u;
     std::memcpy(L.a.group_order, c->group_order, sizeof(L.a.group_order));
@@ -1661,6 +1669,9 @@
         if (P.body == LinBody::gated) return k_lin<0, true, FAST, true>;
         if (P.body == LinBody::stamps) return k_lin<2, true, FAST>;
         if (P.body == LinBody::dump) return k_lin<1, true, FAST>;
+    }
+    if constexpr (!SLICE) {
+        if (P.five) return P.one_wave() ? k_lin<0, true, FAST, false, true, false, false, true> : k_lin<0, true, FAST, false, false, false, false, true>;
     }
     if (P.one_wave()) return k_lin<0, true, FAST, false, true, SLICE, GRIDS>;
     return P.fused() ? k_lin<0, true, FAST, false, false, SLICE, GRIDS> : k_lin<0, false, FAST, false, false, SLICE, GRIDS>;
@@ -1743,12 +1754,17 @@
         if (ce != hipSuccess) { (void)hipStreamSynchronize(c->stream); return bail("copying the debug dump back", ce); }
     }
     c->n_launches += 1; c->n_poses_launched += P.n_poses; c->n_points_launched += (int64_t)P.n_poses * L.n;
-    if (L.uses_state(c)) c->state_valid = true;
+    if (L.uses_state(c)) {
+        if (P.five) c->five_tail = 0;
+        else if (c->opt_search_five == 1 && L.state_was_valid && L.state_was_five) c->five_tail = 2;
+        else if (c->five_tail > 0) c->five_tail -= 1;
+        c->state_valid = true; c->state_five = P.five;
+    }
     S.pending = true; S.plan = P; S.timed = timed; S.seq = seq; S.sync = L.dbg != nullptr;
     S.coded = L.a.count_scale != 0.0;
     if (gated) {
         c->gate_slot = L.slot;
-        c->gate_uses_state = L.uses_state(c); c->gate_state_was_valid = L.state_was_valid;
+        c->gate_uses_state = L.uses_state(c); c->gate_state_was_valid = L.state_was_valid; c->gate_state_was_five = L.state_was_five;
     }
     return DCREG_OK;
 }
@@ -1771,6 +1787,7 @@
     L.key.radius_sq_f = a.radius_sq_f; L.key.cert_r_out = a.cert_r_out; L.key.cert_r_in = a.cert_r_in; L.key.fast_plane = c->opt_fast_plane ? 1 : 0;
     if (L.own() && !gated) {
         const double jump = c->last_pose_valid ? pose_jump(c, L.R9, L.t3, c->last_R, c->last_t) : 1e300;
+        c->last_step = c->hint_unknown ? jump : 0.0;
         if (c->hint_unknown && jump <= 0.5 * c->map.grid.h) c->hint_misalign = c->hint_last;
         if (jump > 0.5 * c->map.grid.h) { c->last_searched = c->n_src; c->last_points = c->last_searched; }
         c->hint_unknown = false;
@@ -1784,7 +1801,7 @@
         if (int rc = stale ? estimate_dispatch_order(c, L.R9, L.t3, a.max_ring) : DCREG_OK) return rc;
     }
     if (L.uses_state(c) && !(L.key == c->state_key)) { c->state_valid = false; c->state_key = L.key; }
-    L.state_was_valid = c->state_valid;
+    L.state_was_valid = c->state_valid; L.state_was_five = c->state_five;
     L.one.state = kNoIdx; L.one.fresh = 1;
     if (L.own()) {
         std::memcpy(L.one.R, L.R9, sizeof(L.one.R)); std::memcpy(L.one.t, L.t3, sizeof(L.one.t));
@@ -2095,6 +2112,9 @@
     else if (k == "team_stamps") c->opt_team_stamps = v != 0.0;
     else if (k == "team_pass") c->opt_team_pass = (int)v;
     else if (k == "advance_min_blocks") c->opt_advance_min_blocks = (int)v;
+    else if (k == "search_five") c->opt_search_five = (int)std::min(std::max(v, 0.0), 2.0);
+    else if (k == "search_five_step") c->opt_search_five_step = std::max(v, 0.0);
+    else if (k == "search_five_frac") c->opt_search_five_frac = std::min(std::max(v, 0.0), 1.0);
     else if (k == "team_search") c->opt_team_max = (int)v;
     else if (k == "spin") c->opt_spin = v != 0.0;
     else if (k == "far_bound") c->opt_far_bound = v != 0.0;
@@ -2437,6 +2457,7 @@
         return DCREG_E_STATE;
     }
     gate_publish(c, c->gate_seq << 1, R, t);
+    c->last_step = c->last_pose_valid ? pose_jump(c, R, t, c->last_R, c->last_t) : 1e300;
     std::memcpy(c->last_R, R, sizeof(c->last_R)); std::memcpy(c->last_t, t, sizeof(c->last_t));
     c->last_pose_valid = true;
     c->gate_slot = -1;
@@ -2449,7 +2470,7 @@
     LinSlot &S = c->slots[c->gate_slot];
     S.pending = false;
     free_tmp(S);
-    if (c->gate_uses_state) c->state_valid = c->gate_state_was_valid;
+    if (c->gate_uses_state) { c->state_valid = c->gate_state_was_valid; c->state_five = c->gate_state_was_five; }
     c->gate_slot = -1;
     return DCREG_OK;
 }
diff --git a/dcreg_amd/csrc/device/context.hpp b/dcreg_amd/csrc/device/context.hpp
--- a/dcreg_amd/csrc/device/context.hpp
+++ b/dcreg_amd/csrc/device/context.hpp
@@ -143,10 +143,11 @@
     bool gate_inside = false;
     bool pass_rows = false;
     bool ordered = false, use_cert = true;
+    bool five = false;
     bool fused() const { return body != LinBody::chunked; }
     bool one_wave() const { return body == LinBody::one_wave; }
     int passes() const { return (int)pass | (one_wave() ? 4 : 0); }
-    int structure() const { return pass_rows ? 2 : pass != LinPass::none ? 1 : 0; }
+    int structure() const { return (pass_rows ? 2 : pass != LinPass::none ? 1 : 0) | (five ? 4 : 0); }
 };
 
 struct LinSlot {
@@ -429,6 +430,7 @@
     int gate_slot = -1;
     bool gate_uses_state = false;
     bool gate_state_was_valid = false;
+    bool gate_state_was_five = false;
     static constexpr int kLinSlots = 2;
     LinSlot slots[kLinSlots];
 
@@ -481,6 +483,12 @@
     DevBuf<unsigned long long> d_team_stamps; uint32_t team_stamps_n = 0;
     DevBuf<uint32_t> d_adv_counts; bool adv_counts_dirty = true;
     int64_t n_advance_launches = 0;
+    int opt_search_five = 1;
+    double opt_search_five_step = 0.04;
+    double opt_search_five_frac = 0.95;
+    bool state_five = false;
+    int five_tail = 0;
+    double last_step = 0.0;
     int opt_team_max = 7;
     bool opt_warm = true;
     int64_t n_launches = 0, n_poses_launched = 0, n_points_launched = 0;
diff --git a/dcreg_amd/csrc/device/kernels.hpp b/dcreg_amd/csrc/device/kernels.hpp
--- a/dcreg_amd/csrc/device/kernels.hpp
+++ b/dcreg_amd/csrc/device/kernels.hpp
@@ -369,7 +369,7 @@
 constexpr int kAdvTile = 1536;
 static_assert(kAdvTile % kLinBlock == 0 && kAdvTile <= 65536, "a tile is a whole number of query blocks; list entries are 16-bit offsets");
 
-template <int MODE, bool FUSED, bool FAST, bool GATE = false, bool ONE = false, bool SLICE = false, bool GRIDS = false>
+template <int MODE, bool FUSED, bool FAST, bool GATE = false, bool ONE = false, bool SLICE = false, bool GRIDS = false, bool FIVE = false>
 static __global__ __launch_bounds__(ONE ? kWave : kLinBlock, kLinOcc) void k_lin(const float4 *__restrict__ src, uint32_t n_src, GridDev g,
                                                           PoseArg pose1, const PoseArg *__restrict__ poses, LinArgs a,
                                                           double *__restrict__ partials, uint32_t n_blocks_x, FinArgs fin,
@@ -380,6 +380,7 @@
     static_assert(!ONE || (MODE == 0 && FUSED && !GATE), "the one-wave instantiation is the fused product launch behind k_gate");
     static_assert(!SLICE || (MODE == 0 && !GATE), "per-pose source slices are batched product launches");
     static_assert(!GRIDS || SLICE, "per-pose target grids come with per-pose source slices");
+    static_assert(!FIVE || (MODE == 0 && FUSED && !GATE && !SLICE), "five-neighbour launches are fused single-pose product launches");
     if constexpr (GRIDS) {
         const PairGrid &pg = grids[grid_ids[blockIdx.y]];
         g = pg.g; a.max_ring = pg.max_ring; a.infl_max_d2 = pg.infl_max_d2;
@@ -448,8 +449,9 @@
     float qx, qy, qz;
     body_to_global(P, (double)s4.x, (double)s4.y, (double)s4.z, qx, qy, qz);
     const float q0x = __uint_as_float(q0[0]), q0y = __uint_as_float(q0[1]), q0z = __uint_as_float(q0[2]);
-    const bool need = have_q && !(CERT && cert_holds(cert, q0x, q0y, q0z, qx, qy, qz));
-    bool refit = have_q && !need && !cert_is_out(cert) && !fit_holds(fitw, q0x, q0y, q0z, qx, qy, qz);
+    const bool need = have_q && !(CERT && cert_holds(cert, q0x, q0y, q0z, qx, qy, qz) &&
+                                  (!FIVE || cert_is_out(cert) || fit_holds(fitw, q0x, q0y, q0z, qx, qy, qz)));
+    bool refit = !FIVE && have_q && !need && !cert_is_out(cert) && !fit_holds(fitw, q0x, q0y, q0z, qx, qy, qz);
     uint32_t stats = 0;
     uint32_t w_search = 0, w_refit = 0;
     uint32_t adv_s = 0, adv_r = 0;
@@ -486,7 +488,7 @@
                 pos6[0] = x.x; pos6[1] = x.y; pos6[2] = x.z; pos6[3] = x.w; pos6[4] = y.x; pos6[5] = y.y;
             }
             bool by_team = false;
-            if (warm && w_search <= (uint32_t)a.team_max) {
+            if (!FIVE && warm && w_search <= (uint32_t)a.team_max) {
                 float tb = 0.f;
                 bool tight = false;
                 if (need && pos6[5] != kNoIdx) tb = team_bound(g, a, pos6, qx, qy, qz, tight);
@@ -502,7 +504,18 @@
                     }
                 }
             }
-            if (!by_team) {
+            if constexpr (FIVE) {
+                Set5 s5;
+                lin_search5<kLinSweep, kLinDepth>(g, runs[wave], a, need, warm, pos6, qx, qy, qz, s5);
+                if (need) {
+                    const bool in5 = s5.pos[4] != kNoIdx && (double)s5.d2[4] < a.radius_sq;
+                    cert = in5 ? 0u : 0x80000000u;
+#pragma unroll
+                    for (int j = 0; j < 5; ++j) pos6[j] = s5.pos[j];
+                    pos6[5] = kNoIdx;
+                    stats = (s5.n_eval & 0xFFFFu) | ((s5.n_shell & 0x7FFFu) << 16);
+                }
+            } else if (!by_team) {
                 Set6 s6;
                 uint32_t c2;
                 lin_search6<kLinSweep, kLinDepth>(g, runs[wave], a, need, warm, pos6, qx, qy, qz, s6, c2);
@@ -523,9 +536,9 @@
         const bool fitnow = set && (need || refit);
         w_refit = (uint32_t)__builtin_popcountll(__builtin_amdgcn_ballot_w64(fitnow && !need));
         if (wave_any(fitnow)) {
-            const bool use6 = fitnow && cert_is_set6(cert);
+            const bool use6 = !FIVE && fitnow && cert_is_set6(cert);
             const bool six = wave_any(use6);
-            const bool presorted = !wave_any(fitnow && !need);
+            const bool presorted = FIVE || !wave_any(fitnow && !need);
             if (fitnow && !need) {
                 const uint4 x = SX[iw];
                 const uint2 y = SY[iw];
@@ -541,10 +554,14 @@
                         const uint32_t o1 = SW3[iw];
                         cert = cert_rebased(cert, __uint_as_float(o0.z), __uint_as_float(o0.w), __uint_as_float(o1), qx, qy, qz);
                     }
+                    if constexpr (FIVE) {
+                        SV0[iw] = make_uint4(cert, kFitNone, __float_as_uint(qx), __float_as_uint(qy));
+                    } else {
                     SV0[iw] = make_uint4(cert, fit.word, __float_as_uint(qx), __float_as_uint(qy));
                     SV1[iw] = dbl2{fit.plane[0], fit.plane[1]};
                     SV2[iw] = dbl2{fit.plane[2], fit.plane[3]};
                     SW3[iw] = __float_as_uint(qz);
+                    }
                 }
             }
         }
@@ -556,7 +573,7 @@
         }
         if (!set && need && keep) {
             SV0[iw] = make_uint4(cert, kFitNone, __float_as_uint(qx), __float_as_uint(qy));
-            SW3[iw] = __float_as_uint(qz);
+            if constexpr (!FIVE) SW3[iw] = __float_as_uint(qz);
         }
     }
     double nrm[3] = {0.0, 0.0, 0.0}, r_pt = 0.0, s_pt = 0.0;
diff --git a/dcreg_amd/csrc/device/search.hpp b/dcreg_amd/csrc/device/search.hpp
--- a/dcreg_amd/csrc/device/search.hpp
+++ b/dcreg_amd/csrc/device/search.hpp
@@ -1,6 +1,7 @@
 #pragma once
 #include <stddef.h>
 #include <stdint.h>
+#include <type_traits>
 #if defined(DCREG_HOST_EMUL)
 #define DCREG_DEVFN inline
 #define DCREG_ON_DEVICE 0
@@ -244,6 +245,21 @@
     }
 };
 
+struct Top5 {
+    static constexpr int K = 5;
+    float d[5];
+    uint32_t n_eval, n_shell;
+    DCREG_DEVFN void init(float bound_f) {
+#pragma unroll
+        for (int i = 0; i < 5; ++i) d[i] = bound_f;
+        n_eval = 0; n_shell = 1;
+    }
+    DCREG_DEVFN void push(float x, uint32_t , uint32_t , bool  = true) {
+        d[4] = med3f(d[3], d[4], x); d[3] = med3f(d[2], d[3], x);
+        d[2] = med3f(d[1], d[2], x); d[1] = med3f(d[0], d[1], x); d[0] = fminf(d[0], x);
+    }
+};
+
 DCREG_DEVFN float dist2_nofma(float qx, float qy, float qz, const float4 &c) {
 #pragma clang fp contract(off)
     typedef float f2 __attribute__((ext_vector_type(2)));
@@ -275,7 +291,7 @@
 }
 
 struct RunList;
-template <class H, bool SWEEP, bool NOTE>
+template <class H, bool SWEEP, bool NOTE, bool INCL = false>
 DCREG_DEVFN void knn_shells(const GridDev &g, RunList &rl, float qx, float qy, float qz, int cx, int cy, int cz,
                                            double fx, double fy, double fz, float bound_f, int max_ring, H &hp);
 
@@ -330,7 +346,7 @@
     }
 }
 
-template <class H, bool NOTE>
+template <class H, bool NOTE, bool INCL = false>
 DCREG_DEVFN void scan_run_deferred(const GridDev &g, RunList &rl, uint32_t s, uint32_t e, float qx, float qy, float qz, H &hp) {
     DCREG_STAT(runs);
     const int tid = threadIdx.x & (kWave - 1);
@@ -352,7 +368,7 @@
         for (int u = 0; u < 4; ++u) {
             const float d2 = dist2_nofma(qx, qy, qz, c[u]);
             const bool valid = p + u < e;
-            const bool pass = valid && d2 < lim;
+            const bool pass = valid && (INCL ? d2 <= lim : d2 < lim);
             hp.n_eval += valid ? 1u : 0u;
             if (pass) { rl.pend[cnt][tid] = PendEntry{__float_as_uint(d2), p + u}; ++cnt; }
             if (NOTE) om = fminf(om, (valid && !pass) ? d2 : __builtin_inff());
@@ -377,7 +393,7 @@
     if (NOTE) hp.note_outside(om);
 }
 
-template <class H, bool SWEEP = false, bool NOTE = true, int DEPTH = 2>
+template <class H, bool SWEEP = false, bool NOTE = true, int DEPTH = 2, bool INCL = false>
 DCREG_DEVFN void knn_search(const GridDev &g, RunList &rl, float qx, float qy, float qz, float bound_f,
                                            int max_ring, H &hp, float infl = 1.f, float cap = __builtin_inff(), bool empty_block = false) {
     hp.init(bound_f, infl, cap);
@@ -483,7 +499,7 @@
                 for (int u = 0; u < W; ++u) {
                     const float d2 = dist2_nofma(qx, qy, qz, sl.c[u]);
                     const bool valid = sl.cp + u < sl.ce;
-                    const bool pass = valid && d2 < lim;
+                    const bool pass = valid && (INCL ? d2 <= lim : d2 < lim);
                     hp.n_eval += valid ? 1u : 0u;
                     if (pass) { rl.pend[cnt][tid] = PendEntry{__float_as_uint(d2), sl.cp + u}; ++cnt; }
                     if (NOTE) om = fminf(om, (valid && !pass) ? d2 : __builtin_inff());
@@ -510,10 +526,10 @@
             hp.note_outside(om);
         }
     }
-    knn_shells<H, SWEEP, NOTE>(g, rl, qx, qy, qz, cx, cy, cz, fx, fy, fz, bound_f, max_ring, hp);
-}
-
-template <class H, bool SWEEP, bool NOTE>
+    knn_shells<H, SWEEP, NOTE, INCL>(g, rl, qx, qy, qz, cx, cy, cz, fx, fy, fz, bound_f, max_ring, hp);
+}
+
+template <class H, bool SWEEP, bool NOTE, bool INCL>
 DCREG_DEVFN void knn_shells(const GridDev &g, RunList &rl, float qx, float qy, float qz, int cx, int cy, int cz,
                                            double fx, double fy, double fz, float bound_f, int max_ring, H &hp) {
     const int nx = g.nx, ny = g.ny, nz = g.nz;
@@ -533,7 +549,7 @@
     auto lookup_scan = [&](int64_t c0, int64_t c1) {
         DCREG_STAT(table_loads); DCREG_STAT(table_loads); DCREG_STAT(faces);
         const uint32_t s_ = g.cell_start[c0], e_ = g.cell_start[c1];
-        if constexpr (SWEEP && H::kDeferred) scan_run_deferred<H, NOTE>(g, rl, s_, e_, qx, qy, qz, hp);
+        if constexpr (SWEEP && H::kDeferred) scan_run_deferred<H, NOTE, INCL>(g, rl, s_, e_, qx, qy, qz, hp);
         else scan_run<H>(g, s_, e_, qx, qy, qz, hp);
     };
     const float frx = (float)(fx - (double)cx), fry = (float)(fy - (double)cy), frz = (float)(fz - (double)cz);
@@ -1057,6 +1073,27 @@
     }
 }
 
+struct Set5 {
+    uint32_t pos[5];
+    float d2[5];
+    uint32_t n_eval, n_shell;
+};
+template <bool SWEEP, int DEPTH = 2>
+DCREG_DEVFN void search5(const GridDev &g, RunList &rl, float qx, float qy, float qz, float bound_f, int max_ring, Set5 &out, bool empty_block = false) {
+    HeapFast<5> hf;
+    knn_search<HeapFast<5>, SWEEP, false, DEPTH, true>(g, rl, qx, qy, qz, bound_f, max_ring, hf, 1.f, __builtin_inff(), empty_block);
+    out.n_eval = hf.n_eval; out.n_shell = hf.n_shell;
+#pragma unroll
+    for (int j = 0; j < 5; ++j) { out.pos[j] = hf.pos[j]; out.d2[j] = hf.d[j]; }
+    if (hf.boundary_tie()) {
+        HeapExact<5> he;
+        knn_search<HeapExact<5>, SWEEP>(g, rl, qx, qy, qz, bound_f, max_ring, he, 1.f, __builtin_inff(), empty_block);
+        out.n_eval += he.n_eval;
+#pragma unroll
+        for (int j = 0; j < 5; ++j) { out.pos[j] = he.pos[j]; out.d2[j] = he.dist(j); }
+    }
+}
+
 DCREG_DEVFN uint32_t make_cert(const Set6 &s, const LinArgs &a) {
     const float a4 = sqrt_approx(s.d2[4]), a5 = sqrt_approx(s.d2[5]), a6 = sqrt_approx(s.lb7);
     const float s_out = a4 * 0.999998f - a.cert_r_out;
@@ -1076,26 +1113,37 @@
     return m2 < s * s;
 }
 
+constexpr float kFiveBoundGrow = 1.3f;
 DCREG_DEVFN float warm_bound6(const GridDev &g, const uint32_t (&oldpos)[6], float qx, float qy, float qz, float bound) {
     float4 pv[6];
 #pragma unroll
-    for (int j = 0; j < 6; ++j) pv[j] = g.pts[oldpos[j]];
+    for (int j = 0; j < 5; ++j) pv[j] = g.pts[oldpos[j]];
+    pv[5] = g.pts[oldpos[5] != kNoIdx ? oldpos[5] : oldpos[4]];
     float m = 0.f;
 #pragma unroll
     for (int j = 0; j < 6; ++j) m = fmaxf(m, dist2_nofma(qx, qy, qz, pv[j]));
+    if (oldpos[5] == kNoIdx) m *= kFiveBoundGrow;
     const float incl = fmaxf(__uint_as_float(__float_as_uint(m) + 1u), 1.17549435e-38f);
     return fminf(bound, incl);
 }
-
-template <bool SWEEP, int DEPTH = 2>
-DCREG_DEVFN void lin_search6(const GridDev &g, RunList &runs, const LinArgs &a, bool have_q, bool warm, const uint32_t (&oldpos)[6],
-                             float qx, float qy, float qz, Set6 &st, uint32_t &cert) {
-    float bound = a.radius_sq_f;
-    if (warm && oldpos[5] != kNoIdx) bound = warm_bound6(g, oldpos, qx, qy, qz, bound);
+DCREG_DEVFN float warm_bound5(const GridDev &g, const uint32_t (&oldpos)[6], float qx, float qy, float qz, float bound) {
+    float4 pv[5];
+#pragma unroll
+    for (int j = 0; j < 5; ++j) pv[j] = g.pts[oldpos[j]];
+    float m = 0.f;
+#pragma unroll
+    for (int j = 0; j < 5; ++j) m = fmaxf(m, dist2_nofma(qx, qy, qz, pv[j]));
+    const float incl = fmaxf(__uint_as_float(__float_as_uint(m) + 1u), 1.17549435e-38f);
+    return fminf(bound, incl);
+}
+
+template <int K>
+DCREG_DEVFN void lin_start_bound(const GridDev &g, const LinArgs &a, bool have_q, float qx, float qy, float qz, float &bound, bool &reach,
+                                 bool &all_in_space) {
     const double fx = ((double)qx - g.ox) * g.inv_h, fy = ((double)qy - g.oy) * g.inv_h, fz = ((double)qz - g.oz) * g.inv_h;
     const double lim = (double)a.max_ring + 1.0;
-    const bool reach = have_q && !(fx < -lim || fy < -lim || fz < -lim || fx > g.nx + lim || fy > g.ny + lim || fz > g.nz + lim);
-    bool all_in_space = false;
+    reach = have_q && !(fx < -lim || fy < -lim || fz < -lim || fx > g.nx + lim || fy > g.ny + lim || fz > g.nz + lim);
+    all_in_space = false;
     if (g.owner) {
         bool far = false;
         uint32_t oc = kNoIdx;
@@ -1117,7 +1165,7 @@
             all_in_space = !wave_any(reach && !in_space);
         }
         if (wave_any(far)) {
-            Top6 hb;
+            typename std::conditional<K == 6, Top6, Top5>::type hb;
             hb.init(bound);
             uint32_t s_ = 0, e_ = 0;
             if (far) {
@@ -1128,7 +1176,7 @@
                 e_ = min(e_, s_ + 48u);
             }
             scan_run<decltype(hb), kProbeBatch>(g, s_, e_, qx, qy, qz, hb);
-            bool more = far && e_ - s_ < 6u && !(hb.d[5] < bound);
+            bool more = far && e_ - s_ < (uint32_t)K && !(hb.d[K - 1] < bound);
             if (wave_any(more)) {
                 uint32_t ox = 0, oy = 0, oz = 0;
                 if (more) { ox = oc % (uint32_t)g.nx; const uint32_t r_ = oc / (uint32_t)g.nx; oy = r_ % (uint32_t)g.ny; oz = r_ / (uint32_t)g.ny; }
@@ -1145,12 +1193,21 @@
                         }
                     }
                     scan_run<decltype(hb), kProbeBatch>(g, s2, e2, qx, qy, qz, hb);
-                    more = far && !(hb.d[5] < bound);
+                    more = far && !(hb.d[K - 1] < bound);
                 }
             }
-            if (far) bound = fminf(bound, fmaxf(__uint_as_float(__float_as_uint(hb.d[5]) + 1u), 1.17549435e-38f));
-        }
-    }
+            if (far) bound = fminf(bound, fmaxf(__uint_as_float(__float_as_uint(hb.d[K - 1]) + 1u), 1.17549435e-38f));
+        }
+    }
+}
+
+template <bool SWEEP, int DEPTH = 2>
+DCREG_DEVFN void lin_search6(const GridDev &g, RunList &runs, const LinArgs &a, bool have_q, bool warm, const uint32_t (&oldpos)[6],
+                             float qx, float qy, float qz, Set6 &st, uint32_t &cert) {
+    float bound = a.radius_sq_f;
+    if (warm && oldpos[4] != kNoIdx) bound = warm_bound6(g, oldpos, qx, qy, qz, bound);
+    bool reach, all_in_space;
+    lin_start_bound<6>(g, a, have_q, qx, qy, qz, bound, reach, all_in_space);
     const float infl = a.prune_infl, cap = a.infl_max_d2 * a.prune_infl;
     bound = fminf(fmaxf(bound, fminf(bound * infl, cap)), a.radius_sq_f);
 #pragma unroll
@@ -1158,6 +1215,19 @@
     st.lb7 = bound; st.n_eval = 0; st.n_shell = 1;
     if (reach) search6<SWEEP, DEPTH>(g, runs, qx, qy, qz, bound, a.max_ring, infl, cap, st, SWEEP && all_in_space);
     cert = make_cert(st, a);
+}
+
+template <bool SWEEP, int DEPTH = 2>
+DCREG_DEVFN void lin_search5(const GridDev &g, RunList &runs, const LinArgs &a, bool have_q, bool warm, const uint32_t (&oldpos)[6],
+                             float qx, float qy, float qz, Set5 &st) {
+    float bound = a.radius_sq_f;
+    if (warm && oldpos[4] != kNoIdx) bound = warm_bound5(g, oldpos, qx, qy, qz, bound);
+    bool reach, all_in_space;
+    lin_start_bound<5>(g, a, have_q, qx, qy, qz, bound, reach, all_in_space);
+#pragma unroll
+    for (int j = 0; j < 5; ++j) { st.pos[j] = kNoIdx; st.d2[j] = bound; }
+    st.n_eval = 0; st.n_shell = 1;
+    if (reach) search5<SWEEP, DEPTH>(g, runs, qx, qy, qz, bound, a.max_ring, st, SWEEP && all_in_space);
 }
 
 
```

Result: faster. 17450, median of 6 (+4.3%).
